# psweens/VAN-GAN

Measured on AMD Instinct MI355X. Metric: train Mvoxels/s (VanGan.train_step, 128^3 bf16), higher is better.
Workload: dtype bf16; 1 GPU; VanGan.train_step, 128x128x128 volumes, batch 1 per GPU (global 1), clDice on, disc noise+dropout on; parallelism=dp1

## Files before the change

### include/vangan_hip.h

```cpp
#ifndef VANGAN_HIP_H
#define VANGAN_HIP_H
#include <stdint.h>
#ifdef __cplusplus
extern "C" {
#endif

typedef void* vg_stream_t;

#define VG_OK 0
#define VG_EINVAL (-1)
#define VG_ELDS (-2)
#define VG_ELAUNCH (-3)

#define VG_ACT_NONE 0
#define VG_ACT_RELU 1
#define VG_ACT_LRELU 2

#define VG_PAD_ZERO 0
#define VG_PAD_REFLECT 1

#define VG_MAX_TAPS 64

#define VG_STRIPES 8

// ... 40 lines not shown
    int32_t Cout;
    const void* wpacked;
    int32_t CK;
    const float* bias;
    const void* res;
    const float* res_scale;
    const float* res_shift;
    int32_t tanh_out;
    void* out;
    int32_t out_f32;
    int32_t accumulate;
    float* out_sums;
    int32_t f32;
    int32_t nclass;
    int32_t cls_tap0[9];
    const void* cls_w[8];
    int32_t cls_ooff[8][3];
    int32_t cls_iters[8][3];
    int32_t wpack;
    int32_t wpack_wmin;
    const struct vg_actnorm_bwd_desc_s* bstat;
    void* scratch;
    int64_t scratch_bytes;
    int32_t wlayout;
    const vg_fin_desc* fin;
    int32_t res_c1;
    const void* wpacked_up;
} vg_conv_desc;
#define VG_SCRATCH_CTR_BYTES 16384

int vg_conv3d(const vg_conv_desc* d, vg_stream_t stream);

int vg_conv3d_lds_bytes(const vg_conv_desc* d);
int vg_conv3d_plan(const vg_conv_desc* d, int32_t* plan4);
int vg_conv3d_thin_np(const vg_conv_desc* d);
int vg_conv3d_variant(const vg_conv_desc* d, char* buf, int buflen);
int vg_set_tuning(const char* key, int value, int reset);

int vg_pack_up_weights(const float* w, int Cin, int Cout, int c_up, void* out, vg_stream_t stream);

int vg_pack_weights(const float* w, int T, int Cin, int Cout, const int32_t* tap_idx_dev, int ntaps,
                    int transpose, int CK, void* out, int out_f32, vg_stream_t stream);
typedef struct {
    const float* w; const int32_t* tap_idx; void* out;
    int32_t Cin, Cout, ntaps, transpose, CK, out_f32;
    int32_t blk0, nblk;
    int32_t bn;
    int32_t pad_;
} vg_pack_item;
int vg_pack_weights_multi(const vg_pack_item* items_dev, int n, int total_blocks, vg_stream_t stream);
int vg_conv3d_dma_bn(const vg_conv_desc* d);
int64_t vg_conv3d_scratch_bytes(const vg_conv_desc* d);
int vg_pack_weights_dma(const float* w, int T, int Cin, int Cout, const int32_t* tap_idx_dev, int ntaps, int transpose, int bn,
                        void* out, vg_stream_t stream);
int vg_packed_ktot(int ntaps, int C, int CK);
int vg_packed_rows(int N);

int vg_conv3d_wgrad(const vg_conv_desc* d, const void* dy, int dy_f32, const int32_t* tap_idx_host,
                    int T_total, float* dw, float* db, float* scratch, int64_t scratch_bytes, vg_stream_t stream);
int vg_conv3d_wgrad_variant(const vg_conv_desc* d, int dy_f32, const int32_t* tap_idx_host, int T_total,
                            int64_t scratch_bytes, char* buf, int buflen);

int vg_in_finalize(const float* sums0, int c0, float count0, const float* sums1, int c1, float count1,
                   const float* gamma, const float* beta, const float* mult, int N, float eps,
                   float* scale, float* shift, float* mean, float* rstd, vg_stream_t stream);

typedef struct vg_actnorm_bwd_desc_s {
    const void* g; int32_t g_padded;
    const void* x; int32_t x_f32;
    const void* x1; int32_t c_x0; int32_t x0_shift;
    int32_t N, D, H, W, C;
    const float* scale; const float* shift;
    const float* mult;
    int32_t act; int32_t norm;
    const float* gamma; const float* mean; const float* rstd;
    float* red;
    void* dx; int32_t dx_f32; int32_t accumulate;
    int32_t dx_cstride, dx_coff;
    int32_t f32;
    float* dgamma;
    float* dbeta;
    int32_t* ticket;
    int32_t alias_n0, alias_shift, pgrad_n, pad_;
} vg_actnorm_bwd_desc;
int vg_actnorm_bwd_stats(const vg_actnorm_bwd_desc* d, vg_stream_t stream);
int vg_actnorm_bwd_apply(const vg_actnorm_bwd_desc* d, vg_stream_t stream);
int vg_actnorm_bwd_apply2(const vg_actnorm_bwd_desc* d1, const vg_actnorm_bwd_desc* d2, vg_stream_t stream);
int vg_actnorm_bwd(const vg_actnorm_bwd_desc* d, vg_stream_t stream);
int vg_stem_short_fwd_workgroups(int N, int64_t S);
int vg_stem_short_fwd(const float* x, int N, int64_t S, int C, const float* w, const float* gamma, const float* beta, float eps, int round16,
                      float* scale, float* shift, double* part, int G, unsigned* ticket, vg_stream_t stream);
int vg_stem_short_bwd_workgroups(int N, int64_t S, int C);
int vg_stem_short_bwd(const void* g, int g_f32, const float* x, int N, int64_t S, int C, const float* w, const float* gamma, float eps,
                      int round16, float* dw, float* dgamma, float* dbeta, double* part, int G, unsigned* ticket, vg_stream_t stream);
int vg_in_param_grads(const float* red, int N, int C, float* dgamma, float* dbeta, vg_stream_t stream);

int vg_concat_bwd(const void* g, int N, int D, int H, int W, int Cu, int Cs, void* dlow, void* dskip,
                  int f32, int accumulate, vg_stream_t stream);

int vg_shortcut_dgrad_concat(const vg_conv_desc* d, void* dlow, void* dskip, int c_low, int accumulate, vg_stream_t stream);
int vg_shortcut_dgrad_concat_norm(const vg_conv_desc* d, const vg_actnorm_bwd_desc* b, void* dlow, void* dskip, int c_low,
                                  int accumulate, vg_stream_t stream);

int vg_affine_add(const void* a, const float* a_scale, const float* a_shift, int a_act, const void* b, const float* b_scale,
                  const float* b_shift, int N, int64_t S, int C, void* out, int f32, vg_stream_t stream);

int vg_bias_grad(const void* dy, int f32, int64_t rows, int C, float* db, vg_stream_t stream);

int vg_pack_cell_weights(const float* w, int C, void* out, vg_stream_t stream);
int vg_cells_fold(const void* cells, int N, int D, int H, int W, float* dx, vg_stream_t stream);

int vg_tanh_bwd(const float* dy, const float* y, float* dpre, int64_t n, vg_stream_t stream);

int vg_minmax(const float* x, int B, int64_t S, float* mm4, vg_stream_t stream);
int vg_minmax_apply(const float* x, const float* mm4, int B, int64_t S, float* y, vg_stream_t stream);
int vg_minmax_bwd(const float* x, const float* y, const float* gy, const float* mm4, int B, int64_t S,
                  float* tmp2, float* dx, vg_stream_t stream);
int vg_bce(const float* t, const float* p, int64_t n, float* acc, float gscale, float* gp, int accumulate,
           vg_stream_t stream);
int vg_mse(const float* a, const float* b, int64_t n, float* acc, float gscale, float* gb, int accumulate,
           vg_stream_t stream);
int vg_mse_const(const void* x, int x_f32, float target, int64_t n, float* acc, float gscale, float* gx,
                 int accumulate, vg_stream_t stream);
int vg_lp_loss(const float* a, const float* b, int64_t n, int p, float* acc, float gscale, float* gb, int accumulate,
               vg_stream_t stream);
int vg_logit_loss(const void* x, int x_f32, float target, int kind, int64_t n, float* acc, float gscale, float* gx,
                  int accumulate, vg_stream_t stream);
int vg_ssim_fwd(const float* t, const float* p, int B, int D, int H, int W, float* acc, float* part,
                vg_stream_t stream);
int vg_ssim_bwd(const float* t, const float* p, const float* part, int B, int D, int H, int W, float gscale,
                float* gp, int accumulate, vg_stream_t stream);

int vg_soft_skel_fwd(const float* img, int B, int D, int H, int W, int iters, float* imgs, float* skels, void* aux,
                     vg_stream_t stream);
int vg_soft_skel_bwd(const float* imgs, const float* skels, const float* gskel, int B, int D, int H, int W,
                     int iters, float* work, float* gimg, const void* aux, vg_stream_t stream);
int vg_cldice_coef(const float* sums7, float w, float alpha, float* coef6, vg_stream_t stream);
int vg_cldice_grads(const float* t, const float* skel_t, const float* coef6, int64_t n, float* gskel_p, float* gp,
                    int accumulate, vg_stream_t stream);
int vg_dot_sums(const float* a, const float* b, int64_t n, float* sums3, vg_stream_t stream);
int vg_axpby(const float* a, float alpha, const float* b, float beta, int64_t n, float* y, int accumulate,
             vg_stream_t stream);

int vg_dense_head_fwd(const float* x, const float* mask, const float* w, const float* b, int N, int n, float* z, vg_stream_t stream);
int vg_dense_head_bwd(const float* x, const float* mask, const float* w, const float* gz, int N, int n, float* dx, float* dw, float* db,
                      vg_stream_t stream);
int vg_wasserstein_terms(const float* z, int B, float inv, float* acc2, float* gz_d, float* gz_g, vg_stream_t stream);

int vg_overlap_add(const float* win, int kx, int ky, int kz, int px, int py, int pz, int x0, int y0, int z0,
                   int X, int Y, int Z, float* pred, float* cnt, vg_stream_t stream);
int vg_divide_crop(const float* pred, const float* cnt, int X, int Y, int Z, int sx, int sy, int sz, int ox, int oy,
                   int oz, float* out, vg_stream_t stream);
int vg_window_gather(const float* vol, int X, int Y, int Z, const int* tab, int B, int kx, int ky, int kz, float* out,
                     vg_stream_t stream);
int vg_window_scatter(const float* win, const int* tab, int B, int kx, int ky, int kz, int px, int py, int pz, const float* wx,
                      const float* wy, const float* wz, int X, int Y, int Z, float* pred, float* cnt, vg_stream_t stream);

int vg_adam_clip(float* w, const float* g, float* m, float* v, const int64_t* seg_off_dev, int T,
                 int64_t total, float* norms, float lr_t, float beta1, float beta2, float eps,
                 float clipnorm, float grad_scale, vg_stream_t stream);

#define VG_SN_MAX_ITEMS 8
#define VG_SN_MAX_PROJ 4
#define VG_SN_MAX_COUT 512
#define VG_SN_SLAB 65536
#define VG_SN_STATE 8
// ... 106 lines not shown
```

### van_gan_amd/_lib.py

```python
from __future__ import annotations

import ctypes as C
import os

import torch

from . import build as _build

VG_MAX_TAPS = 64
SN_STATE, SN_STATE_CUM, SN_MAX_PROJ = 8, 4, 4
ACT_NONE, ACT_RELU, ACT_LRELU = 0, 1, 2
PAD_ZERO, PAD_REFLECT = 0, 1
SCRATCH_CTR_BYTES = 16384

c_void_p, c_int, c_float, c_i64, c_u64 = C.c_void_p, C.c_int32, C.c_float, C.c_int64, C.c_uint64


class ConvDesc(C.Structure):
    _fields_ = [
        ('src0', c_void_p), ('src1', c_void_p), ('c_src0', c_int), ('c_src1', c_int), ('src0_shift', c_int),
        ('src_f32', c_int), ('N', c_int), ('D', c_int), ('H', c_int), ('W', c_int),
        ('in_scale', c_void_p), ('in_shift', c_void_p), ('act', c_int), ('noise', c_void_p), ('noise_pad', c_int),
        ('istr', c_int), ('pad_mode', c_int), ('ntaps', c_int),
        ('tap_d', C.c_int8 * VG_MAX_TAPS), ('tap_h', C.c_int8 * VG_MAX_TAPS), ('tap_w', C.c_int8 * VG_MAX_TAPS),
        ('OD', c_int), ('OH', c_int), ('OW', c_int), ('ostr', c_int), ('ooff_d', c_int), ('ooff_h', c_int),
        ('ooff_w', c_int), ('BD', c_int), ('BH', c_int), ('BW', c_int), ('Cout', c_int),
        ('wpacked', c_void_p), ('CK', c_int), ('bias', c_void_p),
        ('res', c_void_p), ('res_scale', c_void_p), ('res_shift', c_void_p), ('tanh_out', c_int),
        ('out', c_void_p), ('out_f32', c_int), ('accumulate', c_int), ('out_sums', c_void_p), ('f32', c_int),
        ('nclass', c_int), ('cls_tap0', c_int * 9), ('cls_w', c_void_p * 8), ('cls_ooff', (c_int * 3) * 8),
        ('cls_iters', (c_int * 3) * 8), ('wpack', c_int), ('wpack_wmin', c_int), ('bstat', c_void_p),
        ('scratch', c_void_p), ('scratch_bytes', c_i64), ('wlayout', c_int), ('fin', c_void_p), ('res_c1', c_int), ('wpacked_up', c_void_p),
    ]


class FinJob(C.Structure):
    _fields_ = [('gamma', c_void_p), ('beta', c_void_p), ('mult', c_void_p), ('scale', c_void_p), ('shift', c_void_p),
                ('mean', c_void_p), ('rstd', c_void_p), ('c_off', c_int), ('c_tot', c_int)]


class FinDesc(C.Structure):
    _fields_ = [('ticket', c_void_p), ('count', c_float), ('eps', c_float), ('njobs', c_int), ('job', FinJob * 2)]


class PackItem(C.Structure):
    _fields_ = [('w', c_void_p), ('tap_idx', c_void_p), ('out', c_void_p), ('Cin', c_int), ('Cout', c_int), ('ntaps', c_int),
                ('transpose', c_int), ('CK', c_int), ('out_f32', c_int), ('blk0', c_int), ('nblk', c_int), ('bn', c_int), ('pad_', c_int)]


class SnItem(C.Structure):
    _fields_ = [('w', c_void_p), ('u', c_void_p), ('state', c_void_p), ('K', c_int), ('Cout', c_int), ('blk0', c_int), ('nblk', c_int)]


class ActNormBwdDesc(C.Structure):
    _fields_ = [
        ('g', c_void_p), ('g_padded', c_int), ('x', c_void_p), ('x_f32', c_int),
        ('x1', c_void_p), ('c_x0', c_int), ('x0_shift', c_int),
        ('N', c_int), ('D', c_int), ('H', c_int), ('W', c_int), ('C', c_int),
        ('scale', c_void_p), ('shift', c_void_p), ('mult', c_void_p), ('act', c_int), ('norm', c_int),
        ('gamma', c_void_p), ('mean', c_void_p), ('rstd', c_void_p), ('red', c_void_p),
        ('dx', c_void_p), ('dx_f32', c_int), ('accumulate', c_int), ('dx_cstride', c_int), ('dx_coff', c_int),
        ('f32', c_int), ('dgamma', c_void_p), ('dbeta', c_void_p), ('ticket', c_void_p),
        ('alias_n0', c_int), ('alias_shift', c_int), ('pgrad_n', c_int), ('pad_', c_int),
    ]


_SIGS = {
    'vg_version': ([], c_int),
    'vg_storage16': ([], c_int),
    'vg_abi_sizeof': ([c_int], c_int),
    'vg_set_stamp_buffer': ([c_void_p], c_int),
    'vg_conv3d': ([C.POINTER(ConvDesc), c_void_p], c_int),
    'vg_conv3d_lds_bytes': ([C.POINTER(ConvDesc)], c_int),
    'vg_conv3d_plan': ([C.POINTER(ConvDesc), C.POINTER(C.c_int32)], c_int),
    'vg_conv3d_variant': ([C.POINTER(ConvDesc), C.c_char_p, c_int], c_int),
    'vg_conv3d_thin_np': ([C.POINTER(ConvDesc)], c_int),
    'vg_set_tuning': ([C.c_char_p, c_int, c_int], c_int),
    'vg_conv3d_wgrad_variant': ([C.POINTER(ConvDesc), c_int, C.POINTER(c_int), c_int, c_i64, C.c_char_p, c_int], c_int),
    'vg_pack_weights': ([c_void_p, c_int, c_int, c_int, c_void_p, c_int, c_int, c_int, c_void_p, c_int, c_void_p], c_int),
    'vg_pack_weights_multi': ([c_void_p, c_int, c_int, c_void_p], c_int),
    'vg_crop_augment': ([c_void_p] + [c_int] * 13 + [c_void_p, c_void_p], c_int),
    'vg_crop_max': ([c_void_p] + [c_int] * 10 + [c_void_p, c_void_p], c_int),
    'vg_conv3d_dma_bn': ([C.POINTER(ConvDesc)], c_int),
    'vg_conv3d_scratch_bytes': ([C.POINTER(ConvDesc)], c_i64),
    'vg_pack_weights_dma': ([c_void_p, c_int, c_int, c_int, c_void_p, c_int, c_int, c_int, c_void_p, c_void_p], c_int),
    'vg_packed_ktot': ([c_int, c_int, c_int], c_int),
    'vg_packed_rows': ([c_int], c_int),
    'vg_conv3d_wgrad': ([C.POINTER(ConvDesc), c_void_p, c_int, C.POINTER(c_int), c_int, c_void_p, c_void_p, c_void_p, c_i64,
                         c_void_p], c_int),
    'vg_in_finalize': ([c_void_p, c_int, c_float, c_void_p, c_int, c_float, c_void_p, c_void_p, c_void_p, c_int,
                        c_float, c_void_p, c_void_p, c_void_p, c_void_p, c_void_p], c_int),
    'vg_actnorm_bwd_stats': ([C.POINTER(ActNormBwdDesc), c_void_p], c_int),
    'vg_actnorm_bwd_apply': ([C.POINTER(ActNormBwdDesc), c_void_p], c_int),
    'vg_actnorm_bwd_apply2': ([C.POINTER(ActNormBwdDesc), C.POINTER(ActNormBwdDesc), c_void_p], c_int),
    'vg_actnorm_bwd': ([C.POINTER(ActNormBwdDesc), c_void_p], c_int),
    'vg_stem_short_fwd_workgroups': ([c_int, c_i64], c_int),
    'vg_stem_short_fwd': ([c_void_p, c_int, c_i64, c_int, c_void_p, c_void_p, c_void_p, C.c_float, c_int, c_void_p, c_void_p, c_void_p, c_int, c_void_p,
                          c_void_p], c_int),
    'vg_stem_short_bwd_workgroups': ([c_int, c_i64, c_int], c_int),
    'vg_stem_short_bwd': ([c_void_p, c_int, c_void_p, c_int, c_i64, c_int, c_void_p, c_void_p, C.c_float, c_int, c_void_p, c_void_p, c_void_p,
                          c_void_p, c_int, c_void_p, c_void_p], c_int),
    'vg_in_param_grads': ([c_void_p, c_int, c_int, c_void_p, c_void_p, c_void_p], c_int),
    'vg_concat_bwd': ([c_void_p, c_int, c_int, c_int, c_int, c_int, c_int, c_void_p, c_void_p, c_int, c_int, c_void_p], c_int),
    'vg_shortcut_dgrad_concat': ([C.POINTER(ConvDesc), c_void_p, c_void_p, c_int, c_int, c_void_p], c_int),
    'vg_shortcut_dgrad_concat_norm': ([C.POINTER(ConvDesc), C.POINTER(ActNormBwdDesc), c_void_p, c_void_p, c_int, c_int, c_void_p], c_int),
    'vg_affine_add': ([c_void_p, c_void_p, c_void_p, c_int, c_void_p, c_void_p, c_void_p, c_int, c_i64, c_int, c_void_p, c_int, c_void_p], c_int),
    'vg_bias_grad': ([c_void_p, c_int, c_i64, c_int, c_void_p, c_void_p], c_int),
    'vg_pack_cell_weights': ([c_void_p, c_int, c_void_p, c_void_p], c_int),
    'vg_cells_fold': ([c_void_p, c_int, c_int, c_int, c_int, c_void_p, c_void_p], c_int),
    'vg_tanh_bwd': ([c_void_p, c_void_p, c_void_p, c_i64, c_void_p], c_int),
    'vg_minmax': ([c_void_p, c_int, c_i64, c_void_p, c_void_p], c_int),
    'vg_minmax_apply': ([c_void_p, c_void_p, c_int, c_i64, c_void_p, c_void_p], c_int),
    'vg_minmax_bwd': ([c_void_p, c_void_p, c_void_p, c_void_p, c_int, c_i64, c_void_p, c_void_p, c_void_p], c_int),
    'vg_bce': ([c_void_p, c_void_p, c_i64, c_void_p, c_float, c_void_p, c_int, c_void_p], c_int),
    'vg_mse': ([c_void_p, c_void_p, c_i64, c_void_p, c_float, c_void_p, c_int, c_void_p], c_int),
    'vg_mse_const': ([c_void_p, c_int, c_float, c_i64, c_void_p, c_float, c_void_p, c_int, c_void_p], c_int),
    'vg_lp_loss': ([c_void_p, c_void_p, c_i64, c_int, c_void_p, c_float, c_void_p, c_int, c_void_p], c_int),
    'vg_logit_loss': ([c_void_p, c_int, c_float, c_int, c_i64, c_void_p, c_float, c_void_p, c_int, c_void_p], c_int),
    'vg_ssim_fwd': ([c_void_p, c_void_p, c_int, c_int, c_int, c_int, c_void_p, c_void_p, c_void_p], c_int),
    'vg_ssim_bwd': ([c_void_p, c_void_p, c_void_p, c_int, c_int, c_int, c_int, c_float, c_void_p, c_int, c_void_p], c_int),
    'vg_soft_skel_fwd': ([c_void_p, c_int, c_int, c_int, c_int, c_int, c_void_p, c_void_p, c_void_p, c_void_p], c_int),
    'vg_soft_skel_bwd': ([c_void_p, c_void_p, c_void_p, c_int, c_int, c_int, c_int, c_int, c_void_p, c_void_p, c_void_p, c_void_p], c_int),
    'vg_cldice_coef': ([c_void_p, c_float, c_float, c_void_p, c_void_p], c_int),
    'vg_cldice_grads': ([c_void_p, c_void_p, c_void_p, c_i64, c_void_p, c_void_p, c_int, c_void_p], c_int),
    'vg_dense_head_fwd': ([c_void_p, c_void_p, c_void_p, c_void_p, c_int, c_int, c_void_p, c_void_p], c_int),
    'vg_dense_head_bwd': ([c_void_p, c_void_p, c_void_p, c_void_p, c_int, c_int, c_void_p, c_void_p, c_void_p, c_void_p], c_int),
    'vg_wasserstein_terms': ([c_void_p, c_int, c_float, c_void_p, c_void_p, c_void_p, c_void_p], c_int),
    'vg_dot_sums': ([c_void_p, c_void_p, c_i64, c_void_p, c_void_p], c_int),
    'vg_overlap_add': ([c_void_p] + [c_int] * 12 + [c_void_p, c_void_p, c_void_p], c_int),
    'vg_divide_crop': ([c_void_p, c_void_p] + [c_int] * 9 + [c_void_p, c_void_p], c_int),
    'vg_window_gather': ([c_void_p, c_int, c_int, c_int, c_void_p] + [c_int] * 4 + [c_void_p, c_void_p], c_int),
    'vg_window_scatter': ([c_void_p, c_void_p] + [c_int] * 7 + [c_void_p] * 3 + [c_int] * 3 + [c_void_p] * 3, c_int),
    'vg_slice_moments_scratch_bytes': ([c_i64, c_int], c_i64),
    'vg_slice_moments': ([c_void_p, c_int, c_i64, c_int, c_void_p, c_void_p, c_i64, c_void_p], c_int),
    'vg_zscore_slices': ([c_void_p, c_int, c_i64, c_int, c_void_p, c_void_p, c_void_p, c_void_p], c_int),
    'vg_order_stats_scratch_bytes': ([c_i64, c_int], c_i64),
    'vg_order_stats': ([c_void_p, c_i64, C.POINTER(c_i64), c_int, c_void_p, c_void_p, c_i64, c_void_p], c_int),
    'vg_clip_rescale': ([c_void_p, c_i64, c_void_p, C.c_double, C.c_double, c_int, c_void_p, c_void_p, c_void_p], c_int),
    'vg_resample_axis': ([c_void_p, c_i64, c_int, c_i64, c_int, c_void_p, c_void_p, c_void_p, c_void_p], c_int),
    'vg_value_mode_scratch_bytes': ([c_i64], c_i64),
    'vg_value_mode': ([c_void_p, c_i64, c_void_p, c_void_p, c_void_p, c_i64, c_void_p], c_int),
    'vg_label_finish': ([c_void_p, c_i64, c_void_p, c_void_p, c_void_p, c_void_p, c_void_p], c_int),
    'vg_median3': ([c_void_p] + [c_int] * 7 + [c_void_p, c_void_p, c_void_p], c_int),
    'vg_volume_moments_scratch_bytes': ([c_i64], c_i64),
    'vg_volume_moments': ([c_void_p, c_int, c_i64, c_void_p, c_void_p, c_i64, c_void_p], c_int),
    'vg_outlier_limits': ([c_void_p, c_int, c_i64, c_void_p, c_float, c_void_p, c_void_p, c_void_p], c_int),
# ... 81 lines not shown
```

### van_gan_amd/csrc/vg_common.h

```cpp
#pragma once
#include <hip/hip_runtime.h>
#include <stdint.h>
#include "../../include/vangan_hip.h"

typedef __attribute__((ext_vector_type(8))) short bf16x8;
typedef __attribute__((ext_vector_type(4))) short bf16x4;
typedef __attribute__((ext_vector_type(4))) float f32x4;
typedef unsigned short bf16_t;

#define VG_LDS_LIMIT 163840
#define VG_LRELU 0.2f

#ifdef VG_FP16
typedef __attribute__((ext_vector_type(8))) _Float16 vg_h8;
__device__ __forceinline__ float bf2f(bf16_t h) { return (float)__builtin_bit_cast(_Float16, h); }
__device__ __forceinline__ bf16_t f2bf(float f) { return __builtin_bit_cast(unsigned short, (_Float16)f); }
#define VG_MFMA16(a, b, c) __builtin_amdgcn_mfma_f32_16x16x32_f16(__builtin_bit_cast(vg_h8, a), __builtin_bit_cast(vg_h8, b), c, 0, 0, 0)
#define VG_MFMA32(a, b, c) __builtin_amdgcn_mfma_f32_32x32x16_f16(__builtin_bit_cast(vg_h8, a), __builtin_bit_cast(vg_h8, b), c, 0, 0, 0)
#define VG_STORAGE16 "fp16"
#else
__device__ __forceinline__ float bf2f(bf16_t h) { return __uint_as_float(((unsigned)h) << 16); }
__device__ __forceinline__ bf16_t f2bf(float f) {
    __bf16 b = (__bf16)f;
    return __builtin_bit_cast(unsigned short, b);
// ... 36 lines not shown

__device__ __forceinline__ float vg_act(float x, int act) {
    if (act == VG_ACT_RELU) return fmaxf(x, 0.f);
    if (act == VG_ACT_LRELU) return x > 0.f ? x : VG_LRELU * x;
    return x;
}
__device__ __forceinline__ float vg_act_grad(float pre, int act) {
    if (act == VG_ACT_RELU) return pre > 0.f ? 1.f : 0.f;
    if (act == VG_ACT_LRELU) return pre > 0.f ? 1.f : VG_LRELU;
    return 1.f;
}

__device__ __forceinline__ float wave_sum(float v) {
#pragma unroll
    for (int o = 32; o > 0; o >>= 1) v += __shfl_xor(v, o);
    return v;
}
__device__ __forceinline__ float wave_min(float v) {
#pragma unroll
    for (int o = 32; o > 0; o >>= 1) v = fminf(v, __shfl_xor(v, o));
    return v;
}
__device__ __forceinline__ float wave_max(float v) {
#pragma unroll
    for (int o = 32; o > 0; o >>= 1) v = fmaxf(v, __shfl_xor(v, o));
    return v;
}

struct VgFin { unsigned* ticket; float count, eps; int njobs; vg_fin_job job[2]; };
static inline VgFin vg_fin_of(const vg_conv_desc* d) {
    VgFin f; f.ticket = nullptr; f.count = 1.f; f.eps = 0.f; f.njobs = 0;
    if (d->fin && d->out_sums) { f.ticket = d->fin->ticket; f.count = d->fin->count; f.eps = d->fin->eps; f.njobs = d->fin->njobs;
                                 f.job[0] = d->fin->job[0]; f.job[1] = d->fin->job[d->fin->njobs > 1 ? 1 : 0]; }
    return f;
}
__device__ __forceinline__ void vg_fin_one(const VgFin& f, float s, float ss, int n, int c) {
    const float mean = s / f.count;
    float var = ss / f.count - mean * mean;
    var = var < 0.f ? 0.f : var;
    const float rstd = rsqrtf(var + f.eps);
    for (int j = 0; j < f.njobs; ++j) {
        const vg_fin_job& q = f.job[j];
        const int cc = q.c_off + c, i = n * q.c_tot + cc;
        float sc = (q.gamma ? q.gamma[cc] : 1.f) * rstd;
        float sh = (q.beta ? q.beta[cc] : 0.f) - mean * sc;
        if (q.mult) { const float m = q.mult[i]; sc *= m; sh *= m; }
        q.scale[i] = sc; q.shift[i] = sh;
        if (q.mean) q.mean[i] = mean;
        if (q.rstd) q.rstd[i] = rstd;
    }
}
__device__ __forceinline__ void vg_fin_tail(const VgFin& f, const float* sums, int N, int C, unsigned nblocks, int* flag) {
    asm volatile("s_waitcnt vmcnt(0)" ::: "memory");
    __syncthreads();
    if (threadIdx.x == 0)
        *flag = __hip_atomic_fetch_add(f.ticket, 1u, __ATOMIC_RELAXED, __HIP_MEMORY_SCOPE_AGENT) == nblocks - 1u ? 1 : 0;
    __syncthreads();
    if (!*flag) return;
    for (int i = threadIdx.x; i < N * C; i += blockDim.x) {
        const int n = i / C, c = i - n * C;
        float s = 0.f, ss = 0.f;
        for (int t = 0; t < VG_STRIPES; ++t) {
            const float* p = sums + (((size_t)t * N + n) * C + c) * 2;
            s += __hip_atomic_load(p, __ATOMIC_RELAXED, __HIP_MEMORY_SCOPE_AGENT);
            ss += __hip_atomic_load(p + 1, __ATOMIC_RELAXED, __HIP_MEMORY_SCOPE_AGENT);
        }
        vg_fin_one(f, s, ss, n, c);
    }
}
int vg_launch_fin(const vg_conv_desc* d, hipStream_t s);
extern thread_local bool vg_fin_done;

int vg_tune(const char* key, int dflt);
bool vg_dry(const char* fmt, ...) __attribute__((format(printf, 1, 2)));
void vg_dry_begin(char* buf, int n);
void vg_dry_end();

bool vg_dry_on();
static inline void vg_begin() { (void)hipGetLastError(); }
static inline int vg_check_launch() {
    hipError_t e = hipGetLastError();
    return e == hipSuccess ? VG_OK : VG_ELAUNCH;
}
int vg_pointwise_conv(const vg_conv_desc* d, hipStream_t s);
int vg_pointwise_wgrad(const vg_conv_desc* d, const void* dy, int dy_f32, int T_total, float* dw, float* db, float* scratch,
                       int64_t scratch_bytes, hipStream_t s);
int vg_wgrad_dma(const vg_conv_desc* d, const void* dy, int dy_f32, const int32_t* tap_idx_host, int T_total, float* dw, float* db,
                 float* scratch, int64_t scratch_bytes, hipStream_t s);
int vg_wgrad_pw_dma(const vg_conv_desc* d, const void* dy, int dy_f32, int T_total, float* dw, float* db, float* scratch,
                    int64_t scratch_bytes, hipStream_t s);
int vg_wgrad_thin(const vg_conv_desc* d, const void* dy, int dy_f32, const int32_t* tap_idx_host, int T_total, float* dw, float* db,
                  float* scratch, int64_t scratch_bytes, hipStream_t s);
int vg_conv_dma(const vg_conv_desc* d, hipStream_t s, bool* did_stats = nullptr);
void vg_launch_reduce_partials(const float* part, int nb, int n, float* dw, hipStream_t s);
static inline int ilog2_exact(int v) { int l = 0; while ((1 << l) < v) ++l; return l; }
static inline int pow2_ceil(int v) { int p = 1; while (p < v) p <<= 1; return p; }
static inline int64_t cdiv64(int64_t a, int64_t b) { return (a + b - 1) / b; }

template <typename T> struct Raw8;
template <> struct Raw8<bf16_t> { bf16x8 v; };
template <> struct Raw8<float> { f32x4 a, b; };
__device__ __forceinline__ void raw_load(Raw8<bf16_t>& r, const bf16_t* p) { r.v = *(const __attribute__((address_space(1))) bf16x8*)(uintptr_t)p; }
__device__ __forceinline__ void raw_load(Raw8<float>& r, const float* p) {
    const __attribute__((address_space(1))) f32x4* q = (const __attribute__((address_space(1))) f32x4*)(uintptr_t)p;
    r.a = q[0]; r.b = q[1];
}
__device__ __forceinline__ void raw_unpack(const Raw8<bf16_t>& r, float* o) {
#pragma unroll
    for (int j = 0; j < 8; ++j) o[j] = bf2f((bf16_t)r.v[j]);
}
__device__ __forceinline__ void raw_unpack(const Raw8<float>& r, float* o) {
    o[0] = r.a[0]; o[1] = r.a[1]; o[2] = r.a[2]; o[3] = r.a[3]; o[4] = r.b[0]; o[5] = r.b[1]; o[6] = r.b[2]; o[7] = r.b[3];
}


__device__ __forceinline__ void raw_pin(Raw8<bf16_t>& r) { asm volatile("" : "+v"(r.v)); }
__device__ __forceinline__ void raw_pin(Raw8<float>& r) { asm volatile("" : "+v"(r.a), "+v"(r.b)); }
__device__ __forceinline__ void raw_mask(Raw8<bf16_t>& r, bool keep) { if (!keep) r.v = (bf16x8){0, 0, 0, 0, 0, 0, 0, 0}; }
__device__ __forceinline__ void raw_mask(Raw8<float>& r, bool keep) { if (!keep) { r.a = (f32x4){0.f, 0.f, 0.f, 0.f}; r.b = r.a; } }

__device__ __forceinline__ float ld_global(const float* p) { return *(const __attribute__((address_space(1))) float*)(uintptr_t)p; }
__device__ __forceinline__ float ld_global(const bf16_t* p) { return bf2f(*(const __attribute__((address_space(1))) bf16_t*)(uintptr_t)p); }
```

### van_gan_amd/csrc/vg_conv.hip

```cpp
#include "vg_conv_common.h"
#include "vg_dma_common.h"

unsigned long long* g_vg_stamps = nullptr;
extern "C" int vg_set_stamp_buffer(void* p) { g_vg_stamps = (unsigned long long*)p; return VG_OK; }
#define VG_STAMP(slot) do { if (g.stamps && tid == 0 && it < 8) g.stamps[((size_t)(blockIdx.z * gridDim.y + blockIdx.y) * gridDim.x + blockIdx.x) * 64 + it * 8 + (slot)] = __builtin_readcyclecounter(); } while (0)

__device__ __attribute__((aligned(16))) unsigned int vg_zero16[4];
typedef __attribute__((address_space(3))) void lds_void_t;
typedef const __attribute__((address_space(1))) void glb_void_t;

__device__ __forceinline__ void dma_build_cq(const GatherIn& g, int* cq, int tid) {
    const int SU = g.DS >> 4;
    for (int q = tid; q < SU; q += 256) {
        const int hh = q / g.HWp, hw = q - hh * g.HWp;
        cq[q] = (hh < g.HH && hw < g.HW) ? (hh | (hw << 10)) : -1;
    }
}
__device__ __forceinline__ void dma_build_tcol(const GatherIn& g, const int* cq, int* tcol, int oh0, int ow0, int tid) {
    const int SU = g.DS >> 4;
    const int ph0 = oh0 * g.istr + g.tmin_h, pw0 = ow0 * g.istr + g.tmin_w;
    const int sh = g.shift0, Ws0 = g.W >> sh;
    for (int q = tid; q < SU; q += 256) {
        const int e = cq[q];
        int o0 = -1, o1 = -1;
// ... 804 lines not shown
    if (!attr_set) {
        (void)hipFuncSetAttribute((const void*)conv_kernel<T, BN, MSUB, NOISE, WL, DMA, MC, C1>, hipFuncAttributeMaxDynamicSharedMemorySize, VG_LDS_LIMIT);
        attr_set = true;
    }
    const int wg_env = vg_tune("CONV_WGS", 0);
    int per_cu = ((BN / 16) * MSUB >= VG_CONV_MW2) ? 2 : VG_CONV_WAVES;
    if (lds > 0 && VG_LDS_LIMIT / lds < per_cu) per_cu = VG_LDS_LIMIT / lds;
    if (per_cu < 1) per_cu = 1;
    const int wg_target = wg_env > 0 ? wg_env : 256 * per_cu;
    const int tiles = g.tiles_d * g.tiles_h * g.tiles_w;
    const int ny = (k.Cout + BN - 1) / BN;
    const int ncp = MC == 2 ? q.ncls : 1;
    int bx = wg_target / (ny * g.N * ncp); if (bx < 1) bx = 1; if (bx > tiles) bx = tiles;
    int ks = 1;
    const long cells = (long)tiles * ny * g.N;
    const long ks_part_bytes = k.scratch_bytes - VG_SCRATCH_CTR_BYTES;
    if (MC == 0 && !DMA && !WL && k.nchunks > 1 && g.ntaps < VG_MAX_TAPS && bx == tiles && cells <= vg_tune("CONV_KSPLIT_CELLS", 256) && cells <= VG_KS_CELLS) {
        const int cap = vg_tune("CONV_KSPLIT", 8);
        constexpr long SLOTB = 256L * (MSUB * (BN / 16)) * 16;
        for (int c = k.nchunks; c >= 2; --c)
            if (k.nchunks % c == 0 && c <= cap && cells * c <= 1024 && cells * c * SLOTB <= ks_part_bytes) { ks = c; break; }
    }
    if (vg_dry("conv<%s,%d,%d,n%d,wl%d,dma%d,mc%d,c1%d>|walk%d|ch%d|ks%d", sizeof(T) == 4 ? "f32" : "bf16", BN, MSUB, (int)NOISE, (int)WL, (int)DMA,
               MC, (int)C1, tiles > bx ? 1 : 0, k.nchunks > 1 ? 1 : 0, ks)) return VG_OK;
    ConvOut k2 = k;
    k2.ks = ks; k2.ks_part = nullptr; k2.ks_cnt = nullptr;
    if (ks > 1) { k2.ks_cnt = (unsigned*)k.scratch; k2.ks_part = (float*)(k.scratch + VG_SCRATCH_CTR_BYTES); }
    dim3 grid(bx * ncp * ks, ny, g.N);
    hipLaunchKernelGGL((conv_kernel<T, BN, MSUB, NOISE, WL, DMA, MC, C1>), grid, dim3(256), lds, s, g, k2, q);
    if (k2.fin.ticket && k2.sums) vg_fin_done = true;
    return vg_check_launch();
}
template <typename T, int BN, int MSUB, bool NOISE>
static int launch_conv2(const GatherIn& g, const ConvOut& k, const ConvCls& q, int lds, hipStream_t s) {
    if (g.Cin == 1) {
        if (q.ncls > 1) return VG_EINVAL;
        if constexpr (sizeof(T) == 2) { if (k.w_lds) return launch_conv3<T, BN, MSUB, NOISE, true, false, 0, true>(g, k, q, lds, s); }
        return launch_conv3<T, BN, MSUB, NOISE, false, false, 0, true>(g, k, q, lds, s);
    }
    if constexpr (!NOISE) {
        if (q.par) {
            if constexpr (sizeof(T) == 2) { if (k.w_lds) return launch_conv3<T, BN, MSUB, NOISE, true, false, 2>(g, k, q, lds, s); }
            return launch_conv3<T, BN, MSUB, NOISE, false, false, 2>(g, k, q, lds, s);
        }
    }
    if constexpr (sizeof(T) == 2 && !NOISE) {
        if (q.ncls > 1) return k.w_lds ? launch_conv3<T, BN, MSUB, NOISE, true, false, 1>(g, k, q, lds, s)
                                       : launch_conv3<T, BN, MSUB, NOISE, false, false, 1>(g, k, q, lds, s);
        if (k.w_lds && k.dma) return launch_conv3<T, BN, MSUB, NOISE, true, true, 0>(g, k, q, lds, s);
    }
    if (q.ncls > 1) return VG_EINVAL;
    if constexpr (sizeof(T) == 2) { if (k.w_lds) return launch_conv3<T, BN, MSUB, NOISE, true, false, 0>(g, k, q, lds, s); }
    return launch_conv3<T, BN, MSUB, NOISE, false, false, 0>(g, k, q, lds, s);
}
template <typename T, int BN, int MSUB>
static int launch_conv(const GatherIn& g, const ConvOut& k, const ConvCls& q, int lds, hipStream_t s) {
    return g.noise ? launch_conv2<T, BN, MSUB, true>(g, k, q, lds, s) : launch_conv2<T, BN, MSUB, false>(g, k, q, lds, s);
}
template <typename T>
static int dispatch_conv(const GatherIn& g, const ConvOut& k, const ConvCls& q, int BN, int MSUB, int lds, hipStream_t s) {
    if (BN == 16 && MSUB == 8) { if constexpr (sizeof(T) == 2) return launch_conv<T, 16, 8>(g, k, q, lds, s); else return VG_EINVAL; }
    if (BN == 16) return MSUB == 4 ? launch_conv<T, 16, 4>(g, k, q, lds, s) : (MSUB == 2 ? launch_conv<T, 16, 2>(g, k, q, lds, s) : launch_conv<T, 16, 1>(g, k, q, lds, s));
    if (BN == 32) return MSUB == 4 ? launch_conv<T, 32, 4>(g, k, q, lds, s) : (MSUB == 2 ? launch_conv<T, 32, 2>(g, k, q, lds, s) : launch_conv<T, 32, 1>(g, k, q, lds, s));
    return MSUB == 2 ? launch_conv<T, 64, 2>(g, k, q, lds, s) : launch_conv<T, 64, 1>(g, k, q, lds, s);
}

static inline bool thin2_shape(const vg_conv_desc* d, const ConvOut& k, const ConvCls& q) {
    return !d->f32 && d->CK == 16 && d->Cout >= 32 && (d->Cout % 32) == 0 && q.ncls == 1 && d->ntaps == 27;
}

extern "C" int vg_conv3d_thin_np(const vg_conv_desc* d0) {
    vg_begin();
    if (!d0) return 0;
    vg_conv_desc d = *d0; d.CK = 16;
    GatherIn g, g2; ConvOut k; ConvCls q; int BN, MSUB, lds;
    if (fill_conv(&d, g, k, q, BN, MSUB, lds) != VG_OK || !thin2_shape(&d, k, q)) return 0;
    if (fill_gather(&d, g2, 16, 512) != VG_OK || !vg_conv_thin_ok(&d, g2, k, q, 2)) return 0;
    return vg_conv_thin_lds_bytes(g2, 2) <= VG_LDS_LIMIT ? 2 : 0;
}

static int conv3d_impl(const vg_conv_desc* d, vg_stream_t stream, bool& did_stats) {
    if (d && d->wlayout) return vg_conv_dma(d, (hipStream_t)stream, &did_stats);
    if (d && d->out && d->wpacked && d->src0 && !d->res_c1) {
        const int prc = vg_pointwise_conv(d, (hipStream_t)stream);
        if (prc <= 0) return prc;
    }
    GatherIn g; ConvOut k; ConvCls q; int BN, MSUB, lds;
    int rc = fill_conv(d, g, k, q, BN, MSUB, lds);
    if (rc != VG_OK) return rc;
    hipStream_t s = (hipStream_t)stream;
    if (!d->res_c1 && thin2_shape(d, k, q)) {
        GatherIn g2;
        if (fill_gather(d, g2, 16, 512) == VG_OK && vg_conv_thin_ok(d, g2, k, q, 2)) {
            const int trc = vg_launch_conv_thin(g2, k, 2, s, d->bstat ? d->bstat->red : nullptr, did_stats);
            if (trc <= 0 && trc != VG_ELDS) return trc;
        }
    }
    { GatherIn g2; int bn2, ms2, lds2; if (plan_conv32(d, k, q, g2, bn2, ms2, lds2) == VG_OK) return launch_conv32(g2, k, q, bn2, ms2, lds2, s); }
    if (!d->f32 && MSUB == 8 && BN == 16 && vg_conv_thin_ok(d, g, k, q, 1)) {
        const int trc = vg_launch_conv_thin(g, k, 1, s, d->bstat ? d->bstat->red : nullptr, did_stats);
        if (trc <= 0 && trc != VG_ELDS) return trc;
    }
    return d->f32 ? dispatch_conv<float>(g, k, q, BN, MSUB, lds, s) : dispatch_conv<bf16_t>(g, k, q, BN, MSUB, lds, s);
}

thread_local bool vg_fin_done = false;
__global__ void fin_kernel(VgFin f, const float* sums, int N, int C) {
    const int i = blockIdx.x * blockDim.x + threadIdx.x;
    if (i >= N * C) return;
    const int n = i / C, c = i - n * C;
    float s = 0.f, ss = 0.f;
    for (int t = 0; t < VG_STRIPES; ++t) { const float* p = sums + (((size_t)t * N + n) * C + c) * 2; s += p[0]; ss += p[1]; }
    vg_fin_one(f, s, ss, n, c);
}
int vg_launch_fin(const vg_conv_desc* d, hipStream_t s) {
    const VgFin f = vg_fin_of(d);
    if (!f.njobs) return VG_OK;
    const int total = d->N * d->Cout;
    hipLaunchKernelGGL(fin_kernel, dim3((total + 255) / 256), dim3(256), 0, s, f, (const float*)d->out_sums, d->N, d->Cout);
    return vg_check_launch();
}
static int fin_check(const vg_conv_desc* d) {
    const vg_fin_desc* f = d->fin;
    if (!f) return VG_OK;
    if (!d->out_sums || !f->ticket || f->njobs < 1 || f->njobs > 2 || !(f->count > 0.f)) return VG_EINVAL;
    for (int j = 0; j < f->njobs; ++j) {
        const vg_fin_job& q = f->job[j];
        if (!q.scale || !q.shift || q.c_off < 0 || q.c_off + d->Cout > q.c_tot) return VG_EINVAL;
    }
    return VG_OK;
}

extern "C" int vg_conv3d(const vg_conv_desc* d, vg_stream_t stream) {
    vg_begin();
    if (!d) return VG_EINVAL;
    if (fin_check(d) != VG_OK) return VG_EINVAL;
    vg_fin_done = false;
    const vg_actnorm_bwd_desc* b = d->bstat;
    if (b) {
        const int pd = b->g_padded ? 2 : 0;
        if (b->g != d->out || !b->norm || !b->red || !b->x || !b->mean || !b->rstd || b->f32 || d->f32 || d->out_f32 || d->accumulate
            || b->N != d->N || b->C != d->Cout || b->D + pd != d->BD || b->H + pd != d->BH || b->W + pd != d->BW)
            return VG_EINVAL;
    }
    bool did_stats = false;
    int rc = conv3d_impl(d, stream, did_stats);
    if (rc == VG_OK && d->fin && !vg_fin_done && !vg_dry_on()) rc = vg_launch_fin(d, (hipStream_t)stream);
    if (rc != VG_OK || !b || vg_dry_on()) return rc;
    if (did_stats) return rc;
    return vg_actnorm_bwd_stats(b, stream);
}

__global__ void pack_weights_kernel(const float* __restrict__ w, int Cin, int Cout, const int* __restrict__ tap_idx,
                                    int ntaps, int transpose, int CK, int kc_pad, int Ktot, int rows_pad,
                                    void* __restrict__ out, int out_f32) {
    const size_t total = (size_t)rows_pad * Ktot;
    const int NR = transpose ? Cin : Cout;
    const int C = transpose ? Cout : Cin;
    for (size_t i = (size_t)blockIdx.x * blockDim.x + threadIdx.x; i < total; i += (size_t)gridDim.x * blockDim.x) {
        const int row = (int)(i / Ktot), k = (int)(i % Ktot);
        const int chunk = k / kc_pad, kl = k % kc_pad;
        const int tap = kl / CK, ch = chunk * CK + kl % CK;
        float v = 0.f;
        if (row < NR && tap < ntaps && ch < C) {
            const int ts = tap_idx[tap];
            v = transpose ? w[((size_t)ts * Cin + row) * Cout + ch] : w[((size_t)ts * Cin + ch) * Cout + row];
        }
// ... 144 lines not shown
```

### van_gan_amd/csrc/vg_elem.hip

```cpp
#include "vg_common.h"
#include <stdlib.h>

__global__ void in_finalize_kernel(const float* sums0, int c0, float cnt0, const float* sums1, int c1, float cnt1,
                                   const float* gamma, const float* beta, const float* mult, int N, float eps,
                                   float* scale, float* shift, float* mean_o, float* rstd_o) {
    const int C = c0 + c1;
    const int i = blockIdx.x * blockDim.x + threadIdx.x;
    if (i >= N * C) return;
    const int n = i / C, c = i % C;
    float s = 0.f, ss = 0.f, cnt;
    if (c < c0) {
        for (int t = 0; t < VG_STRIPES; ++t) { s += sums0[(((size_t)t * N + n) * c0 + c) * 2]; ss += sums0[(((size_t)t * N + n) * c0 + c) * 2 + 1]; }
        cnt = cnt0;
    } else {
        for (int t = 0; t < VG_STRIPES; ++t) { s += sums1[(((size_t)t * N + n) * c1 + (c - c0)) * 2]; ss += sums1[(((size_t)t * N + n) * c1 + (c - c0)) * 2 + 1]; }
        cnt = cnt1;
    }
    const float mean = s / cnt;
    float var = ss / cnt - mean * mean;
    var = var < 0.f ? 0.f : var;
    const float rstd = rsqrtf(var + eps);
    float sc = (gamma ? gamma[c] : 1.f) * rstd;
    float sh = (beta ? beta[c] : 0.f) - mean * sc;
    if (mult) { const float m = mult[i]; sc *= m; sh *= m; }
    scale[i] = sc; shift[i] = sh;
    if (mean_o) mean_o[i] = mean;
    if (rstd_o) rstd_o[i] = rstd;
}

extern "C" int vg_in_finalize(const float* sums0, int c0, float count0, const float* sums1, int c1, float count1,
                              const float* gamma, const float* beta, const float* mult, int N, float eps,
                              float* scale, float* shift, float* mean, float* rstd, vg_stream_t stream) {
    vg_begin();
    if (!sums0 || c0 < 1 || c1 < 0 || (c1 > 0 && !sums1) || !scale || !shift || N < 1) return VG_EINVAL;
    const int total = N * (c0 + c1);
    hipLaunchKernelGGL(in_finalize_kernel, dim3((total + 255) / 256), dim3(256), 0, (hipStream_t)stream, sums0, c0,
                       count0, sums1, c1, count1, gamma, beta, mult, N, eps, scale, shift, mean, rstd);
    return vg_check_launch();
}

struct ANB {
    const void* g; int g_padded;
    const void* x; int x_f32;
    const void* x1; int c_x0, x0_shift;
    int N, D, H, W, C;
    const float* scale; const float* shift; const float* mult;
    int act, norm;
    const float* gamma; const float* mean; const float* rstd;
    float* red;
    int* ticket; float* dgamma; float* dbeta;
    void* dx; int dx_f32, accumulate, dx_cstride, dx_coff;
    int gpc, vpb;
    int alias_n0, alias_sh, pgrad_n;
};
__device__ __forceinline__ int anb_nx(const ANB& p, int n) { return (p.alias_n0 > 0 && n >= p.alias_n0) ? n - p.alias_sh : n; }

template <int VEC> struct ChanK { float sc[VEC], sh[VEC], mu[VEC], rs[VEC], ml[VEC]; };
__device__ __forceinline__ void ldvec(const float* p, float* o, int n) {
    if (n == 8) {
        const __attribute__((address_space(1))) f32x4* q = (const __attribute__((address_space(1))) f32x4*)(uintptr_t)p;
        const f32x4 a = q[0], b = q[1];
        o[0] = a[0]; o[1] = a[1]; o[2] = a[2]; o[3] = a[3]; o[4] = b[0]; o[5] = b[1]; o[6] = b[2]; o[7] = b[3];
    } else o[0] = *p;
}
template <int VEC>
__device__ __forceinline__ void load_chank(const ANB& p, int n, int c, ChanK<VEC>& k) {
    const int nc = anb_nx(p, n) * p.C + c;
#pragma unroll
    for (int j = 0; j < VEC; ++j) { k.sc[j] = 1.f; k.sh[j] = 0.f; k.mu[j] = 0.f; k.rs[j] = 0.f; k.ml[j] = 1.f; }
    if (p.scale) { ldvec(p.scale + nc, k.sc, VEC); ldvec(p.shift + nc, k.sh, VEC); }
    if (p.norm) { ldvec(p.mean + nc, k.mu, VEC); ldvec(p.rstd + nc, k.rs, VEC); }
    if (p.mult) ldvec(p.mult + nc, k.ml, VEC);
}

template <typename T, int VEC> struct RawV;
template <typename T> struct RawV<T, 8> { Raw8<T> r; };
template <typename T> struct RawV<T, 1> { float r; };
template <typename T> __device__ __forceinline__ void rawv_load(RawV<T, 8>& o, const T* p) { raw_load(o.r, p); }
template <typename T> __device__ __forceinline__ void rawv_load(RawV<T, 1>& o, const T* p) { o.r = ld_global(p); }
template <typename T> __device__ __forceinline__ void rawv_unpack(const RawV<T, 8>& o, float* v) { raw_unpack(o.r, v); }
template <typename T> __device__ __forceinline__ void rawv_unpack(const RawV<T, 1>& o, float* v) { v[0] = o.r; }

template <typename T, int VEC, int UB, typename F>
__device__ __forceinline__ void anb_walk_from(const ANB& p, int n, int c, int v, const int stride, const ChanK<VEC>& ck, F&& consume) {
    const int S = p.D * p.H * p.W;
    if (v >= S) return;
    int w = v % p.W, t0 = v / p.W; int h = t0 % p.H, d = t0 / p.H;
    const int sw = stride % p.W, t1 = stride / p.W; const int sh_ = t1 % p.H, sd = t1 / p.H;
    const int PH = p.H + 2, PW = p.W + 2;
    const T* gp = (const T*)p.g + (p.g_padded ? (size_t)n * (p.D + 2) * PH * PW * p.C : (size_t)n * S * p.C) + c;
    const bool need_x = p.act != VG_ACT_NONE || p.norm;
    const bool cat0 = p.x1 && c < p.c_x0;
    const int xs = p.x1 ? p.x0_shift : 0;
    const int Hs = p.H >> xs, Ws = p.W >> xs;
    const int cx = p.x1 ? (cat0 ? p.c_x0 : p.C - p.c_x0) : p.C;
    const T* xp = nullptr;
    const int nx = anb_nx(p, n);
    if (VEC == 8) xp = p.x1 ? (cat0 ? (const T*)p.x + (size_t)nx * (p.D >> xs) * Hs * Ws * cx + c : (const T*)p.x1 + (size_t)nx * S * cx + (c - p.c_x0))
                            : (const T*)p.x + (size_t)nx * S * cx + c;
    const void* x1p = (const char*)p.x + (size_t)nx * S * (p.x_f32 ? 4 : 2);
    for (; v < S; v += UB * stride) {
        RawV<T, VEC> gr[UB], xr[UB];
        float x1v[UB];
        int vv[UB], dd[UB], hh[UB], ww[UB];
#pragma unroll
        for (int k = 0; k < UB; ++k) {
            const bool ok = v + k * stride < S;
            vv[k] = ok ? v + k * stride : -1;
            dd[k] = d; hh[k] = h; ww[k] = w;
            const int vc = ok ? v + k * stride : v;
            const int dc = ok ? d : dd[0], hc = ok ? h : hh[0], wc = ok ? w : ww[0];
            const size_t gi = p.g_padded ? ((size_t)((dc + 1) * PH + hc + 1) * PW + wc + 1) * p.C : (size_t)vc * p.C;
            rawv_load(gr[k], gp + gi);
            if (need_x) {
                if (VEC == 8) {
                    const size_t xi = cat0 ? ((size_t)((dc >> xs) * Hs + (hc >> xs)) * Ws + (wc >> xs)) * cx : (size_t)vc * cx;
                    rawv_load(xr[k], xp + xi);
                } else {
                    x1v[k] = p.x_f32 ? ld_global((const float*)x1p + vc) : ld_global((const bf16_t*)x1p + vc);
                }
            }
            w += sw; if (w >= p.W) { w -= p.W; ++h; }
            h += sh_; if (h >= p.H) { h -= p.H; ++d; }
            d += sd;
        }
#pragma unroll
        for (int k = 0; k < UB; ++k) {
            if (vv[k] < 0) continue;
            float g[VEC], x[VEC];
            rawv_unpack(gr[k], g);
            if (need_x) { if (VEC == 8) rawv_unpack(xr[k], x); else x[0] = x1v[k]; }
            if (p.g_padded) {
                const int dk = dd[k], hk = hh[k], wk = ww[k];
                const bool dhb = dk == 1 || dk == p.D - 2 || hk == 1 || hk == p.H - 2;
                const bool wb = wk == 1 || wk == p.W - 2;
                if (dhb) {
                    const int md = dk == 1 ? 0 : (dk == p.D - 2 ? p.D + 1 : -1);
                    const int mh = hk == 1 ? 0 : (hk == p.H - 2 ? p.H + 1 : -1);
                    const int mw = wk == 1 ? 0 : (wk == p.W - 2 ? p.W + 1 : -1);
                    const int md2 = (dk == 1 && dk == p.D - 2) ? p.D + 1 : -1;
                    const int mh2 = (hk == 1 && hk == p.H - 2) ? p.H + 1 : -1;
                    const int mw2 = (wk == 1 && wk == p.W - 2) ? p.W + 1 : -1;
#pragma unroll
                    for (int a = 0; a < 3; ++a)
#pragma unroll
                        for (int b = 0; b < 3; ++b)
#pragma unroll
                            for (int e = 0; e < 3; ++e) {
                                if ((a | b | e) == 0) continue;
                                const int qd = a == 0 ? dk + 1 : (a == 1 ? md : md2);
                                const int qh = b == 0 ? hk + 1 : (b == 1 ? mh : mh2);
                                const int qw = e == 0 ? wk + 1 : (e == 1 ? mw : mw2);
                                if ((qd | qh | qw) < 0) continue;
                                const size_t idx = ((size_t)(qd * PH + qh) * PW + qw) * p.C;
                                if (VEC == 8) {
                                    float r[8]; load8<T>(gp + idx, r);
#pragma unroll
                                    for (int j = 0; j < 8; ++j) g[j] += r[j];
                                } else g[0] += ld1<T>(gp + idx);
                            }
                } else if (wb) {
                    const size_t rowi = (size_t)((dk + 1) * PH + hk + 1) * PW;
                    float r[VEC];
                    if (wk == 1) {
                        if (VEC == 8) load8<T>(gp + rowi * p.C, r); else r[0] = ld1<T>(gp + rowi * p.C);
#pragma unroll
                        for (int j = 0; j < VEC; ++j) g[j] += r[j];
                    }
                    if (wk == p.W - 2) {
                        if (VEC == 8) load8<T>(gp + (rowi + p.W + 1) * p.C, r); else r[0] = ld1<T>(gp + (rowi + p.W + 1) * p.C);
#pragma unroll
                        for (int j = 0; j < VEC; ++j) g[j] += r[j];
                    }
                }
            }
            float dn[VEC], xh[VEC];
            const float slope = p.act == VG_ACT_RELU ? 0.f : (p.act == VG_ACT_LRELU ? VG_LRELU : 1.f);
#pragma unroll
            for (int j = 0; j < VEC; ++j) {
                float gv = g[j] * ck.ml[j];
                if (need_x) {
                    const float pre = x[j] * ck.sc[j] + ck.sh[j];
                    gv *= (pre > 0.f || p.act == VG_ACT_NONE) ? 1.f : slope;
                    xh[j] = (x[j] - ck.mu[j]) * ck.rs[j];
                } else xh[j] = 0.f;
                dn[j] = gv;
            }
            consume(vv[k], dn, xh);
        }
    }
}

template <typename T, int VEC, int UB, typename F>
__device__ __forceinline__ void anb_walk(const ANB& p, int n, int c, int vl, const ChanK<VEC>& ck, F&& consume) {
    anb_walk_from<T, VEC, UB>(p, n, c, (int)(blockIdx.x * p.vpb + vl), (int)(gridDim.x * p.vpb), ck, consume);
}

template <typename T, int VEC>
__global__ __launch_bounds__(256) void actnorm_stats_kernel(const ANB p) {
    __shared__ float part[16 * 256];
    __shared__ float red[512 * 2];
    const int n = blockIdx.y;
    const int tid = threadIdx.x;
    const int nthr = p.gpc * p.vpb;
    const int cg = tid % p.gpc, vl = tid / p.gpc;
    float s0[VEC], s1[VEC];
#pragma unroll
    for (int j = 0; j < VEC; ++j) { s0[j] = 0.f; s1[j] = 0.f; }
    if (tid < nthr) {
        ChanK<VEC> ck;
        load_chank<VEC>(p, n, cg * VEC, ck);
        anb_walk<T, VEC, 4>(p, n, cg * VEC, vl, ck, [&](int, const float* dn, const float* xh) {
#pragma unroll
            for (int j = 0; j < VEC; ++j) { s0[j] += dn[j]; s1[j] += dn[j] * xh[j]; }
        });
    }
#pragma unroll
    for (int j = 0; j < VEC; ++j) { part[(2 * j) * 256 + tid] = tid < nthr ? s0[j] : 0.f; part[(2 * j + 1) * 256 + tid] = tid < nthr ? s1[j] : 0.f; }
    __syncthreads();
    for (int o = tid; o < p.C * 2; o += 256) {
        const int ch = o >> 1, mom = o & 1;
        const int g8 = ch / VEC, j = ch - g8 * VEC;
        const float* src = part + (2 * j + mom) * 256 + g8;
        float a = 0.f;
        for (int t = 0; t < p.vpb; ++t) a += src[t * p.gpc];
        red[o] = a;
    }
    __syncthreads();
    const int stripe = blockIdx.x & (VG_STRIPES - 1);
    float* dst = p.red + ((size_t)stripe * p.N + n) * p.C * 2;
    for (int i = tid; i < p.C * 2; i += 256) atomicAdd(&dst[i], red[i]);
}

template <typename T, int VEC>
__device__ __forceinline__ void actnorm_apply_body(const ANB& p, const int bx, const int gx) {
    const int n = blockIdx.y;
    const int tid = threadIdx.x;
    const int nthr = p.gpc * p.vpb;
    if (tid >= nthr) return;
    const int cg = tid % p.gpc, vl = tid / p.gpc;
    const int S = p.D * p.H * p.W;
    const int c = cg * VEC;
    float k0[VEC], k1[VEC], k2[VEC];
#pragma unroll
    for (int j = 0; j < VEC; ++j) { k0[j] = 1.f; k1[j] = 0.f; k2[j] = 0.f; }
    if (p.norm) {
        const int nc = n * p.C + c;
        const size_t total = (size_t)p.N * p.C * 2;
        float gm[VEC], rs[VEC], r[2 * VEC];
        ldvec(p.gamma + c, gm, VEC); ldvec(p.rstd + anb_nx(p, n) * p.C + c, rs, VEC);
#pragma unroll
        for (int j = 0; j < 2 * VEC; ++j) r[j] = 0.f;
#pragma unroll
        for (int t = 0; t < VG_STRIPES; ++t) {
            float q[2 * VEC];
            ldvec(p.red + t * total + (size_t)nc * 2, q, VEC);
            if (VEC == 8) ldvec(p.red + t * total + (size_t)nc * 2 + 8, q + 8, VEC); else q[1] = p.red[t * total + (size_t)nc * 2 + 1];
#pragma unroll
            for (int j = 0; j < 2 * VEC; ++j) r[j] += q[j];
        }
        if (p.dgamma && bx == 0 && vl == 0 && (p.pgrad_n <= 0 || n < p.pgrad_n)) {
#pragma unroll
            for (int j = 0; j < VEC; ++j) { atomicAdd(&p.dbeta[c + j], r[2 * j]); atomicAdd(&p.dgamma[c + j], r[2 * j + 1]); }
        }
        const float cnt = (float)S;
#pragma unroll
        for (int j = 0; j < VEC; ++j) { const float gr = gm[j] * rs[j]; k0[j] = gr; k1[j] = gr * r[2 * j] / cnt; k2[j] = gr * r[2 * j + 1] / cnt; }
    }
    ChanK<VEC> ck;
    load_chank<VEC>(p, n, c, ck);
    anb_walk_from<T, VEC, 4>(p, n, c, bx * p.vpb + vl, gx * p.vpb, ck, [&](int v, const float* dn, const float* xh) {
        float o[VEC];
#pragma unroll
        for (int j = 0; j < VEC; ++j) o[j] = k0[j] * dn[j] - k1[j] - k2[j] * xh[j];
        const size_t oidx = ((size_t)n * S + v) * p.dx_cstride + p.dx_coff + c;
        if (p.dx_f32) {
            float* q = (float*)p.dx + oidx;
#pragma unroll
            for (int j = 0; j < VEC; ++j) q[j] = p.accumulate ? q[j] + o[j] : o[j];
        } else if (VEC == 8) {
            bf16_t* q = (bf16_t*)p.dx + oidx;
            if (p.accumulate) {
                float old[8]; load8<bf16_t>(q, old);
#pragma unroll
                for (int j = 0; j < 8; ++j) o[j] += old[j];
            }
            store8<bf16_t>(q, o);
        } else {
            bf16_t* q = (bf16_t*)p.dx + oidx;
            q[0] = f2bf(p.accumulate ? bf2f(q[0]) + o[0] : o[0]);
        }
    });
}
template <typename T, int VEC>
__global__ __launch_bounds__(256) void actnorm_apply_kernel(const ANB p) { actnorm_apply_body<T, VEC>(p, (int)blockIdx.x, (int)gridDim.x); }
template <typename T, int VEC>
__global__ __launch_bounds__(256) void actnorm_apply2_kernel(const ANB p1, const ANB p2, const int g1) {
    if ((int)blockIdx.x < g1) actnorm_apply_body<T, VEC>(p1, (int)blockIdx.x, g1);
    else actnorm_apply_body<T, VEC>(p2, (int)blockIdx.x - g1, (int)gridDim.x - g1);
}

static int fill_anb(const vg_actnorm_bwd_desc* d, ANB& p, bool apply) {
    if (!d || !d->g || d->N < 1 || d->C < 1) return VG_EINVAL;
    if (d->C != 1 && (d->C % 8)) return VG_EINVAL;
    if (d->x_f32 && d->C != 1 && !d->f32) return VG_EINVAL;
    if ((d->act != VG_ACT_NONE || d->norm) && !d->x) return VG_EINVAL;
    if (d->norm && (!d->mean || !d->rstd || !d->red)) return VG_EINVAL;
    if (apply && (!d->dx || (d->norm && !d->gamma))) return VG_EINVAL;
    if (d->g_padded && (d->D < 2 || d->H < 2 || d->W < 2)) return VG_EINVAL;
    if (d->x1 && (d->C == 1 || (d->c_x0 % 8) || d->c_x0 < 8 || d->c_x0 >= d->C)) return VG_EINVAL;
    p.g = d->g; p.g_padded = d->g_padded; p.x = d->x; p.x_f32 = (d->x_f32 || d->f32) ? 1 : 0;
    p.x1 = d->x1; p.c_x0 = d->c_x0; p.x0_shift = d->x1 ? (d->x0_shift ? 1 : 0) : 0;
    p.N = d->N; p.D = d->D; p.H = d->H; p.W = d->W; p.C = d->C;
    p.scale = d->scale; p.shift = d->shift; p.mult = d->mult; p.act = d->act; p.norm = d->norm;
    p.gamma = d->gamma; p.mean = d->mean; p.rstd = d->rstd; p.red = d->red;
    p.ticket = d->ticket; p.dgamma = (d->dgamma && d->dbeta) ? d->dgamma : nullptr; p.dbeta = d->dbeta;
    p.dx = d->dx; p.dx_f32 = (d->dx_f32 || d->f32) ? 1 : 0; p.accumulate = d->accumulate;
    p.dx_cstride = d->dx_cstride > 0 ? d->dx_cstride : d->C; p.dx_coff = d->dx_coff;
    p.alias_n0 = d->alias_n0; p.alias_sh = d->alias_shift; p.pgrad_n = d->pgrad_n;
    if (d->alias_n0 < 0 || (d->alias_n0 > 0 && (d->alias_shift < 1 || d->alias_shift > d->alias_n0 || d->alias_n0 >= d->N)) || d->pgrad_n < 0) return VG_EINVAL;
    p.gpc = d->C == 1 ? 1 : d->C / 8;
    if (p.gpc > 256 || d->C > 512) return VG_EINVAL;
    p.vpb = 256 / p.gpc;
    if (!p.dx_f32 && d->C != 1 && ((p.dx_cstride % 8) || (p.dx_coff % 8))) return VG_EINVAL;
    return VG_OK;
}
static dim3 anb_grid(const ANB& p, bool stats = false) {
    const int S = p.D * p.H * p.W;
    int bx = (S + p.vpb - 1) / p.vpb;
    const int cap_total = vg_tune("ANB_GRID_CAP", 767), cap_stats = vg_tune("ANB_STATS_CAP", 511);
    int cap = (stats ? cap_stats : cap_total) / (p.N > 0 ? p.N : 1);
    if (cap < 1) cap = 1;
    if (bx > cap) bx = cap;
    return dim3(bx, p.N);
}

extern "C" int vg_actnorm_bwd_stats(const vg_actnorm_bwd_desc* d, vg_stream_t stream) {
    vg_begin();
    ANB p; int rc = fill_anb(d, p, false);
    if (rc != VG_OK) return rc;
    if (!p.red) return VG_EINVAL;
    if (d->f32) {
        if (p.C == 1) hipLaunchKernelGGL((actnorm_stats_kernel<float, 1>), anb_grid(p, true), dim3(256), 0, (hipStream_t)stream, p);
        else hipLaunchKernelGGL((actnorm_stats_kernel<float, 8>), anb_grid(p, true), dim3(256), 0, (hipStream_t)stream, p);
    } else {
        if (p.C == 1) hipLaunchKernelGGL((actnorm_stats_kernel<bf16_t, 1>), anb_grid(p, true), dim3(256), 0, (hipStream_t)stream, p);
        else hipLaunchKernelGGL((actnorm_stats_kernel<bf16_t, 8>), anb_grid(p, true), dim3(256), 0, (hipStream_t)stream, p);
    }
    return vg_check_launch();
}
extern "C" int vg_actnorm_bwd_apply(const vg_actnorm_bwd_desc* d, vg_stream_t stream) {
    vg_begin();
    ANB p; int rc = fill_anb(d, p, true);
    if (rc != VG_OK) return rc;
    if (d->f32) {
        if (p.C == 1) hipLaunchKernelGGL((actnorm_apply_kernel<float, 1>), anb_grid(p), dim3(256), 0, (hipStream_t)stream, p);
        else hipLaunchKernelGGL((actnorm_apply_kernel<float, 8>), anb_grid(p), dim3(256), 0, (hipStream_t)stream, p);
    } else {
        if (p.C == 1) hipLaunchKernelGGL((actnorm_apply_kernel<bf16_t, 1>), anb_grid(p), dim3(256), 0, (hipStream_t)stream, p);
        else hipLaunchKernelGGL((actnorm_apply_kernel<bf16_t, 8>), anb_grid(p), dim3(256), 0, (hipStream_t)stream, p);
    }
    return vg_check_launch();
}

extern "C" int vg_actnorm_bwd_apply2(const vg_actnorm_bwd_desc* d1, const vg_actnorm_bwd_desc* d2, vg_stream_t stream) {
    vg_begin();
    ANB p1, p2;
    int rc = fill_anb(d1, p1, true); if (rc != VG_OK) return rc;
    rc = fill_anb(d2, p2, true); if (rc != VG_OK) return rc;
    if (!vg_tune("ANB_APPLY2", 1) || d1->N != d2->N || (d1->f32 != 0) != (d2->f32 != 0) || d1->C == 1 || d2->C == 1) {
        rc = vg_actnorm_bwd_apply(d1, stream);
        return rc != VG_OK ? rc : vg_actnorm_bwd_apply(d2, stream);
    }
    const dim3 g1 = anb_grid(p1), g2 = anb_grid(p2);
    const dim3 grid(g1.x + g2.x, g1.y);
    if (d1->f32) hipLaunchKernelGGL((actnorm_apply2_kernel<float, 8>), grid, dim3(256), 0, (hipStream_t)stream, p1, p2, (int)g1.x);
    else hipLaunchKernelGGL((actnorm_apply2_kernel<bf16_t, 8>), grid, dim3(256), 0, (hipStream_t)stream, p1, p2, (int)g1.x);
    return vg_check_launch();
}

extern "C" int vg_actnorm_bwd(const vg_actnorm_bwd_desc* d, vg_stream_t stream) {
    if (d && d->norm) { const int rc = vg_actnorm_bwd_stats(d, stream); if (rc != VG_OK) return rc; }
    return vg_actnorm_bwd_apply(d, stream);
}

__global__ void in_param_grads_kernel(const float* red, int N, int C, float* dgamma, float* dbeta) {
    const int c = blockIdx.x * blockDim.x + threadIdx.x;
    if (c >= C) return;
    float a = 0.f, b = 0.f;
    for (int n = 0; n < N * VG_STRIPES; ++n) { a += red[((size_t)n * C + c) * 2]; b += red[((size_t)n * C + c) * 2 + 1]; }
    dbeta[c] += a; dgamma[c] += b;
}
template <typename T>
__global__ __launch_bounds__(256) void stem_short_bwd_kernel(const T* g, const float* x, int N, int64_t S, int C, const float* w, const float* gamma,
                                                             float eps, int round16, float* dw, float* dgamma, float* dbeta, double* part,
                                                             unsigned* ticket) {
    __shared__ float sm[4][8][18];
    __shared__ double fin[256][4];
    __shared__ int last;
    const int gpc = C >> 3, vpb = 256 / gpc, tid = threadIdx.x, cg = tid % gpc, vl = tid / gpc, n = blockIdx.y, G = gridDim.x, NV = 2 * C + 2;
    float r0[8], t[8], sx = 0.f, sxx = 0.f;
#pragma unroll
    for (int j = 0; j < 8; ++j) { r0[j] = 0.f; t[j] = 0.f; }
    const T* gn = g + (size_t)n * S * C + cg * 8;
    const float* xn = x + (size_t)n * S;
    constexpr int UN = 8;
    const int64_t vstep = (int64_t)G * vpb;
    int64_t v = (int64_t)blockIdx.x * vpb + vl;
    for (; v + (UN - 1) * vstep < S; v += UN * vstep) {
        Raw8<T> raw[UN]; float xv[UN];
#pragma unroll
        for (int u = 0; u < UN; ++u) { raw_load(raw[u], gn + (v + u * vstep) * C); xv[u] = ld_global(xn + v + u * vstep); }
#pragma unroll
        for (int u = 0; u < UN; ++u) {
            float gv[8];
            raw_unpack(raw[u], gv);
#pragma unroll
            for (int j = 0; j < 8; ++j) { r0[j] += gv[j]; t[j] = fmaf(gv[j], xv[u], t[j]); }
            sx += xv[u]; sxx = fmaf(xv[u], xv[u], sxx);
        }
    }
    for (; v < S; v += vstep) {
        float gv[8];
        load8<T>(gn + v * C, gv);
        const float xv = xn[v];
#pragma unroll
        for (int j = 0; j < 8; ++j) { r0[j] += gv[j]; t[j] = fmaf(gv[j], xv, t[j]); }
        sx += xv; sxx = fmaf(xv, xv, sxx);
    }
    float d[18];
#pragma unroll
    for (int j = 0; j < 8; ++j) { d[j] = r0[j]; d[8 + j] = t[j]; }
    d[16] = sx; d[17] = sxx;
    for (int o = 32; o >= gpc; o >>= 1) {
#pragma unroll
        for (int k = 0; k < 18; ++k) d[k] += __shfl_xor(d[k], o);
    }
    const int lane = tid & 63, wv = tid >> 6;
    if (lane < gpc) {
#pragma unroll
        for (int k = 0; k < 18; ++k) sm[wv][lane][k] = d[k];
    }
    __syncthreads();
    if (tid < NV) {
        int cgi, k;
        if (tid < C) { cgi = tid >> 3; k = tid & 7; }
        else if (tid < 2 * C) { cgi = (tid - C) >> 3; k = 8 + ((tid - C) & 7); }
        else { cgi = 0; k = 16 + tid - 2 * C; }
        __hip_atomic_store(part + ((size_t)n * G + blockIdx.x) * NV + tid,
                           (((double)sm[0][cgi][k] + (double)sm[1][cgi][k]) + (double)sm[2][cgi][k]) + (double)sm[3][cgi][k], __ATOMIC_RELAXED,
                           __HIP_MEMORY_SCOPE_AGENT);
    }
    asm volatile("s_waitcnt vmcnt(0)" ::: "memory");
    __syncthreads();
    if (tid == 0) last = __hip_atomic_fetch_add(ticket, 1u, __ATOMIC_RELAXED, __HIP_MEMORY_SCOPE_AGENT) == (unsigned)(N * G - 1) ? 1 : 0;
    __syncthreads();
    if (!last) return;
    auto ald = [](const double* q) { return __hip_atomic_load(q, __ATOMIC_RELAXED, __HIP_MEMORY_SCOPE_AGENT); };
// ... 544 lines not shown
```

### van_gan_amd/csrc/vg_pointwise.hip

```cpp
#include "vg_common.h"
#include "vg_c1k3.h"
#include <stdlib.h>

namespace {

struct PW {
    const void* x; int x_f32;
    const float* scale; const float* shift; int act;
    const void* w; int kc_pad, CK;
    const float* bias;
    void* out; int out_f32, accumulate, tanh_out;
    float* sums;
    const void* dy; int dy_f32;
    float* dw; float* db;
    int N, C; int64_t S;
    VgFin fin;
};

__device__ __forceinline__ float pw_slope(int act) { return act == VG_ACT_RELU ? 0.f : (act == VG_ACT_LRELU ? VG_LRELU : 1.f); }
__device__ __forceinline__ float ld_single(const void* p, int f32, int64_t i) {
    return f32 ? ld_global((const float*)p + i) : ld_global((const bf16_t*)p + i);
}

template <typename T, int G>
__global__ __launch_bounds__(256) void pw_cto1_kernel(const PW p) {
    const int n = blockIdx.y;
    float wv[G * 8], sc[G * 8], sf[G * 8];
#pragma unroll
    for (int c = 0; c < G * 8; ++c) {
        wv[c] = ld1<T>((const T*)p.w + (c / p.CK) * p.kc_pad + (c % p.CK));
        sc[c] = p.scale ? p.scale[n * p.C + c] : 1.f;
        sf[c] = p.scale ? p.shift[n * p.C + c] : 0.f;
    }
    const float slope = pw_slope(p.act), b = p.bias ? p.bias[0] : 0.f;
    const T* xb = (const T*)p.x + (size_t)n * p.S * p.C;
    const int64_t stride = (int64_t)gridDim.x * 256;
    float s1 = 0.f, s2 = 0.f;
    for (int64_t v = (int64_t)blockIdx.x * 256 + threadIdx.x; v < p.S; v += 2 * stride) {
        Raw8<T> r[2][G];
#pragma unroll
        for (int k = 0; k < 2; ++k) {
            const int64_t vv = v + k * stride < p.S ? v + k * stride : v;
#pragma unroll
            for (int g = 0; g < G; ++g) raw_load(r[k][g], xb + vv * p.C + g * 8);
        }
#pragma unroll
        for (int k = 0; k < 2; ++k) {
            if (v + k * stride >= p.S) continue;
            float a = b;
#pragma unroll
            for (int g = 0; g < G; ++g) {
                float x[8]; raw_unpack(r[k][g], x);
#pragma unroll
                for (int j = 0; j < 8; ++j) {
                    float y = x[j] * sc[g * 8 + j] + sf[g * 8 + j];
                    y = fmaxf(y, y * slope);
                    a += rnd<T>(y) * wv[g * 8 + j];
                }
            }
            const size_t o = (size_t)n * p.S + v + k * stride;
            if (p.tanh_out && !p.accumulate) a = tanhf(a);
            if (p.out_f32) { float* q = (float*)p.out + o; a = p.accumulate ? *q + a : a; *q = a; }
            else { bf16_t* q = (bf16_t*)p.out + o; const bf16_t h = f2bf(p.accumulate ? bf2f(*q) + a : a); *q = h; a = bf2f(h); }
            s1 += a; s2 += a * a;
        }
    }
    if (p.sums) {
        __shared__ float red[8];
#pragma unroll
        for (int o = 32; o > 0; o >>= 1) { s1 += __shfl_xor(s1, o); s2 += __shfl_xor(s2, o); }
        if ((threadIdx.x & 63) == 0) { red[(threadIdx.x >> 6) * 2] = s1; red[(threadIdx.x >> 6) * 2 + 1] = s2; }
        __syncthreads();
        if (threadIdx.x < 2) {
            const int stripe = blockIdx.x & (VG_STRIPES - 1);
            atomicAdd(&p.sums[((size_t)stripe * gridDim.y + n) * 2 + threadIdx.x],
                      red[threadIdx.x] + red[2 + threadIdx.x] + red[4 + threadIdx.x] + red[6 + threadIdx.x]);
        }
    }
}

template <typename T>
__global__ __launch_bounds__(256) void pw_1toc_kernel(const PW p) {
    __shared__ float part[16 * 256];
    const int n = blockIdx.y, tid = threadIdx.x;
    const int gpc = p.C >> 3, vpb = 256 / gpc;
    const int cg = tid % gpc, vl = tid / gpc;
    const bool live = tid < gpc * vpb;
    float wv[8], bv[8], s1[8], s2[8];
#pragma unroll
    for (int j = 0; j < 8; ++j) {
        wv[j] = live ? ld1<T>((const T*)p.w + (size_t)(cg * 8 + j) * p.kc_pad) : 0.f;
        bv[j] = (live && p.bias) ? p.bias[cg * 8 + j] : 0.f;
        s1[j] = 0.f; s2[j] = 0.f;
    }
    const float sc = p.scale ? p.scale[n] : 1.f, sf = p.scale ? p.shift[n] : 0.f, slope = pw_slope(p.act);
    const int64_t xoff = (int64_t)n * p.S;
    T* ob = (T*)p.out + (size_t)n * p.S * p.C + cg * 8;
    const int64_t stride = (int64_t)gridDim.x * vpb;
    if (live)
    for (int64_t v = (int64_t)blockIdx.x * vpb + vl; v < p.S; v += 4 * stride) {
        float xs[4]; Raw8<T> old[4];
#pragma unroll
        for (int k = 0; k < 4; ++k) {
            const int64_t vv = v + k * stride < p.S ? v + k * stride : v;
            xs[k] = ld_single(p.x, p.x_f32, xoff + vv);
            if (p.accumulate) raw_load(old[k], ob + vv * p.C);
        }
#pragma unroll
        for (int k = 0; k < 4; ++k) {
            if (v + k * stride >= p.S) continue;
            float y = xs[k] * sc + sf;
            y = rnd<T>(fmaxf(y, y * slope));
            float o[8];
#pragma unroll
            for (int j = 0; j < 8; ++j) o[j] = y * wv[j] + bv[j];
            if (p.accumulate) {
                float q[8]; raw_unpack(old[k], q);
#pragma unroll
                for (int j = 0; j < 8; ++j) o[j] += q[j];
            }
            store8<T>(ob + (v + k * stride) * p.C, o);
#pragma unroll
            for (int j = 0; j < 8; ++j) { const float r = rnd<T>(o[j]); s1[j] += r; s2[j] += r * r; }
        }
    }
    if (!p.sums) return;
#pragma unroll
    for (int j = 0; j < 8; ++j) { part[(2 * j) * 256 + tid] = live ? s1[j] : 0.f; part[(2 * j + 1) * 256 + tid] = live ? s2[j] : 0.f; }
    __syncthreads();
    const int stripe = blockIdx.x & (VG_STRIPES - 1);
    float* dst = p.sums + ((size_t)stripe * gridDim.y + n) * p.C * 2;
    for (int o = tid; o < p.C * 2; o += 256) {
        const int ch = o >> 1, mom = o & 1, g8 = ch >> 3, j = ch & 7;
        const float* src = part + (2 * j + mom) * 256 + g8;
        float a = 0.f;
        for (int t = 0; t < vpb; ++t) a += src[t * gpc];
        atomicAdd(&dst[o], a);
    }
    if (p.fin.ticket) vg_fin_tail(p.fin, p.sums, gridDim.y, p.C, gridDim.x * gridDim.y, (int*)part);
}

template <typename T, int GI>
__global__ __launch_bounds__(256) void pw_ctoc_kernel(const PW p, int Cin, int Ktot) {
    const int n = blockIdx.y, tid = threadIdx.x;
    const int gpc = p.C >> 3, vpb = 256 / gpc;
    const int cg = tid % gpc, vl = tid / gpc;
    if (tid >= gpc * vpb) return;
    float wv[GI * 8][8], bv[8];
#pragma unroll
    for (int k = 0; k < GI * 8; ++k)
#pragma unroll
        for (int j = 0; j < 8; ++j)
            wv[k][j] = ld1<T>((const T*)p.w + (size_t)(cg * 8 + j) * Ktot + (k / p.CK) * p.kc_pad + (k % p.CK));
#pragma unroll
    for (int j = 0; j < 8; ++j) bv[j] = p.bias ? p.bias[cg * 8 + j] : 0.f;
    const T* xb = (const T*)p.x + (size_t)n * p.S * Cin;
    T* ob = (T*)p.out + (size_t)n * p.S * p.C + cg * 8;
    const int64_t stride = (int64_t)gridDim.x * vpb;
    for (int64_t v = (int64_t)blockIdx.x * vpb + vl; v < p.S; v += 2 * stride) {
        Raw8<T> xr[2][GI], old[2];
#pragma unroll
        for (int k = 0; k < 2; ++k) {
            const int64_t vv = v + k * stride < p.S ? v + k * stride : v;
#pragma unroll
            for (int g = 0; g < GI; ++g) raw_load(xr[k][g], xb + vv * Cin + g * 8);
            if (p.accumulate) raw_load(old[k], ob + vv * p.C);
        }
#pragma unroll
        for (int k = 0; k < 2; ++k) {
            if (v + k * stride >= p.S) continue;
            float o[8];
#pragma unroll
            for (int j = 0; j < 8; ++j) o[j] = bv[j];
#pragma unroll
            for (int g = 0; g < GI; ++g) {
                float x[8]; raw_unpack(xr[k][g], x);
#pragma unroll
                for (int e = 0; e < 8; ++e)
#pragma unroll
                    for (int j = 0; j < 8; ++j) o[j] += x[e] * wv[g * 8 + e][j];
            }
            if (p.accumulate) {
                float q[8]; raw_unpack(old[k], q);
#pragma unroll
                for (int j = 0; j < 8; ++j) o[j] += q[j];
            }
            store8<T>(ob + (v + k * stride) * p.C, o);
        }
    }
}

struct PWG {
    const bf16_t* x0; const bf16_t* x1; int c0, c1, Cin, sh;
    const bf16_t* w; int Ktot, CK, kc_pad;
    const float* bias; bf16_t* out; float* sums;
    int N, ID, IH, IW, OD, OH, OW, istr;
    int BD, BH, BW, ostr, od0, oh0, ow0;
    int Cout; int SO;
    unsigned long long* stamps;
    bf16_t* dlow; bf16_t* dskip; int sc0, sacc;
    const bf16_t* ng; const bf16_t* nx0; const bf16_t* nx1;
    const float* n_scale; const float* n_shift; const float* n_mean; const float* n_rstd; const float* n_gamma; const float* n_mult;
    VgFin fin;
    const float* n_red; float* n_dgamma; float* n_dbeta; int n_act;
};
}
extern unsigned long long* g_vg_stamps;
// ... 716 lines not shown
        if (!nb_->norm || !nb_->g_padded || nb_->f32 || nb_->x_f32 || !nb_->g || !nb_->x || !nb_->x1 || !nb_->x0_shift || nb_->c_x0 != c_low) return 1;
        if (nb_->C != d->Cout || nb_->N != d->N || nb_->D != d->D || nb_->H != d->H || nb_->W != d->W || !nb_->gamma || !nb_->mean || !nb_->rstd || !nb_->red) return 1;
        if (d->D < 4 || d->H < 4 || d->W < 4 || d->D > 1023 || d->H > 1023 || d->W > 1023) return 1;
    }
    if (c_low < 16 || (c_low % 16) || c_low >= d->Cout) return 1;
    if (d->istr != 1 || d->ostr != 1 || d->ooff_d || d->ooff_h || d->ooff_w || d->BD != d->OD || d->BH != d->OH || d->BW != d->OW
        || d->OD != d->D || d->OH != d->H || d->OW != d->W || ((d->D | d->H | d->W) & 1)) return 1;
    const int64_t SO = (int64_t)d->OD * d->OH * d->OW;
    if (SO < 8 || SO > (1 << 30)) return 1;
    const int KS = (Cin + 31) / 32, NB = d->Cout / 16;
    if (!((KS == 1 && (NB == 3 || NB == 6)) || (KS == 2 && NB == 6))) return 1;
    PWG p = {};
    p.x0 = (const bf16_t*)d->src0; p.x1 = p.x0; p.c0 = Cin; p.c1 = 1; p.Cin = Cin; p.sh = 0;
    p.w = (const bf16_t*)d->wpacked; p.CK = d->CK; p.kc_pad = ((d->CK + 31) / 32) * 32; p.Ktot = ((Cin + d->CK - 1) / d->CK) * p.kc_pad;
    p.bias = nullptr; p.out = (bf16_t*)d->out; p.sums = nullptr;
    p.N = d->N; p.ID = d->D; p.IH = d->H; p.IW = d->W; p.OD = d->OD; p.OH = d->OH; p.OW = d->OW; p.istr = 1;
    p.BD = d->BD; p.BH = d->BH; p.BW = d->BW; p.ostr = 1;
    p.Cout = d->Cout; p.SO = (int)SO; p.stamps = g_vg_stamps;
    p.dlow = (bf16_t*)dlow; p.dskip = (bf16_t*)dskip; p.sc0 = c_low; p.sacc = acc;
    if (nb_) {
        p.ng = (const bf16_t*)nb_->g; p.nx0 = (const bf16_t*)nb_->x; p.nx1 = (const bf16_t*)nb_->x1;
        p.n_scale = nb_->scale; p.n_shift = nb_->shift; p.n_mean = nb_->mean; p.n_rstd = nb_->rstd; p.n_gamma = nb_->gamma; p.n_mult = nb_->mult;
        p.n_red = nb_->red; p.n_dgamma = (nb_->dgamma && nb_->dbeta) ? nb_->dgamma : nullptr; p.n_dbeta = nb_->dbeta; p.n_act = nb_->act;
    }
    const int MS = (KS * NB <= 2) ? 4 : 2;
    const int64_t nwt = (SO + MS * 16 - 1) / (MS * 16);
    int64_t b = (nwt + 3) / 4;
    const int capt = vg_tune("PW_GEMM_CAP", 2047);
    const int64_t cap = (capt / d->N) > 0 ? (capt / d->N) : 1;
    if (b > cap) b = cap;
    if (vg_dry("pw_gemm_split<%d,%d,n%d>", KS, NB, nb_ ? 1 : 0)) return VG_OK;
    const bool ok = nb_ ? pwg_launch_split<2>(KS, NB, dim3((int)b, d->N), s, p) : pwg_launch_split<1>(KS, NB, dim3((int)b, d->N), s, p);
    return ok ? vg_check_launch() : 1;
}

int pw_wgrad_cc(const vg_conv_desc* d, const void* dy, int dy_f32, int T_total, float* dw, float* db, float* scratch,
                int64_t scratch_bytes, hipStream_t s) {
    if (!pw_enabled() || !vg_tune("PW_WGRAD_CC", 1)) return 1;
    if (T_total != 1 || d->ntaps != 1 || d->tap_d[0] || d->tap_h[0] || d->tap_w[0] || d->noise || d->wpack || d->nclass > 1) return 1;
    if (d->f32 || d->src_f32 || dy_f32 || d->in_scale || d->act != VG_ACT_NONE) return 1;
    const int Cin = d->c_src0 + d->c_src1;
    if (Cin < 8 || (Cin % 8) || (d->c_src1 && (d->c_src0 % 8)) || d->Cout < 16 || (d->Cout % 16)) return 1;
    if (d->c_src1 && !d->src1) return 1;
    if (d->src0_shift && ((d->D | d->H | d->W) & 1)) return 1;
    if (d->istr < 1 || (d->OD - 1) * d->istr >= d->D || (d->OH - 1) * d->istr >= d->H || (d->OW - 1) * d->istr >= d->W) return 1;
    const int64_t SO = (int64_t)d->OD * d->OH * d->OW;
    if (SO < 1 || SO > (1 << 30)) return 1;
    PWW p = {};
    p.gin = Cin / 8; p.roles = p.gin * (d->Cout / 16);
    if (p.roles > vg_tune("PW_WGRAD_ROLES", 16)) return 1;
    p.rp = pow2_ceil(p.roles); p.vpb = 256 / p.rp;
    p.x0 = (const bf16_t*)d->src0; p.x1 = (const bf16_t*)(d->c_src1 ? d->src1 : d->src0); p.c0 = d->c_src0; p.c1 = d->c_src1 ? d->c_src1 : 1;
    p.Cin = Cin; p.sh = d->src0_shift ? 1 : 0; p.dy = (const bf16_t*)dy; p.Cout = d->Cout;
    p.N = d->N; p.ID = d->D; p.IH = d->H; p.IW = d->W; p.OD = d->OD; p.OH = d->OH; p.OW = d->OW; p.istr = d->istr; p.SO = (int)SO;
    p.dw = dw; p.db = db; p.dw_elems = Cin * d->Cout;
    int64_t b = (SO + (int64_t)p.vpb * 8 - 1) / ((int64_t)p.vpb * 8);
    const int capt = vg_tune("PW_WGRAD_CAP", 511);
    const int64_t cap = (capt / d->N) > 0 ? (capt / d->N) : 1;
    if (b > cap) b = cap;
    if (b < 1) b = 1;
    const int nslab = (int)b * d->N;
    p.part = (nslab > 4 && scratch && (int64_t)nslab * p.dw_elems * 4 <= scratch_bytes) ? scratch : nullptr;
    if (vg_dry("pw_wgrad_cc<r%d>|part%d", p.roles, p.part ? 1 : 0)) return VG_OK;
    hipLaunchKernelGGL(pw_wgrad_cc_kernel, dim3((int)b, d->N), dim3(256), 0, s, p);
    if (p.part) vg_launch_reduce_partials(p.part, nslab, p.dw_elems, dw, s);
    return vg_check_launch();
}

}

extern "C" int vg_shortcut_dgrad_concat(const vg_conv_desc* d, void* dlow, void* dskip, int c_low, int accumulate, vg_stream_t stream) {
    vg_begin();
    if (!d || !d->src0 || !d->out || !d->wpacked || !dlow || !dskip) return VG_EINVAL;
    return pw_gemm_split(d, nullptr, dlow, dskip, c_low, accumulate, (hipStream_t)stream);
}
extern "C" int vg_shortcut_dgrad_concat_norm(const vg_conv_desc* d, const vg_actnorm_bwd_desc* b, void* dlow, void* dskip, int c_low,
                                             int accumulate, vg_stream_t stream) {
    vg_begin();
    if (!d || !b || !d->src0 || !d->wpacked || !dlow || !dskip) return VG_EINVAL;
    if (!vg_tune("PW_SPLIT_NORM", 1)) return 1;
    return pw_gemm_split(d, b, dlow, dskip, c_low, accumulate, (hipStream_t)stream);
}

int vg_pointwise_conv(const vg_conv_desc* d, hipStream_t s) {
    if (pw_enabled() && !d->res && !d->tanh_out && !d->accumulate && d->ostr == 1 && !d->ooff_d && !d->ooff_h && !d->ooff_w
        && d->BD == d->OD && d->BH == d->OH && d->BW == d->OW && !(d->out_f32 && !d->f32)) {
        { const int mrc = c1m_fwd(d, s); if (mrc <= 0) return mrc; }
        C1K3 c;
        if (c1k3_fill(d, c)) {
            c.w = d->wpacked; c.bias = d->bias; c.out = d->out; c.sums = d->out_sums;
            c.fin = vg_fin_of(d);
            const int qpb = 256 / (c.C >> 3);
            int64_t b = ((int64_t)c.D * c.H * c.W4 + qpb - 1) / qpb;
            const int64_t cap = (2047 / d->N) > 0 ? (2047 / d->N) : 1;
            if (b > cap) b = cap;
            const dim3 grid((int)b, d->N);
            if (vg_dry("c1k3_fwd<%s,%s>", d->f32 ? "f32" : "bf16", d->src_f32 ? "f32" : "bf16")) return VG_OK;
            if (d->f32) {
                if (d->src_f32) hipLaunchKernelGGL((c1k3_fwd_kernel<float, float>), grid, dim3(256), 0, s, c);
                else hipLaunchKernelGGL((c1k3_fwd_kernel<float, bf16_t>), grid, dim3(256), 0, s, c);
            } else {
                if (d->src_f32) hipLaunchKernelGGL((c1k3_fwd_kernel<bf16_t, float>), grid, dim3(256), 0, s, c);
                else hipLaunchKernelGGL((c1k3_fwd_kernel<bf16_t, bf16_t>), grid, dim3(256), 0, s, c);
            }
            if (c.sums && c.fin.ticket) vg_fin_done = true;
            return vg_check_launch();
        }
    }
    { const int grc = pw_gemm_conv(d, s); if (grc <= 0) return grc; }
    if (!pw_shape_ok(d) || d->res) return 1;
    if (d->ostr != 1 || d->ooff_d || d->ooff_h || d->ooff_w || d->BD != d->OD || d->BH != d->OH || d->BW != d->OW) return 1;
    if (d->tanh_out && d->accumulate) return 1;
    const int Cin = d->c_src0;
    PW p = {};
    p.x = d->src0; p.x_f32 = d->src_f32; p.scale = d->in_scale; p.shift = d->in_shift; p.act = d->act;
    p.w = d->wpacked; p.CK = d->CK; p.kc_pad = ((d->CK + 31) / 32) * 32;
    p.bias = d->bias; p.out = d->out; p.out_f32 = (d->out_f32 || d->f32) ? 1 : 0; p.accumulate = d->accumulate; p.tanh_out = d->tanh_out;
    p.sums = d->out_sums; p.N = d->N; p.S = (int64_t)d->D * d->H * d->W;
    if (d->Cout == 1 && Cin >= 8 && Cin <= 32 && (Cin % 8) == 0) {
        p.C = Cin;
        const dim3 grid(pw_blocks((p.S + 1) / 2, d->N), d->N);
        if (vg_dry("pw_cto1<%s,%d>", d->f32 ? "f32" : "bf16", Cin / 8 > 4 ? 4 : Cin / 8)) return VG_OK;
#define PW_CTO1(T)                                                                                                      \
        switch (Cin / 8) {                                                                                              \
            case 1: hipLaunchKernelGGL((pw_cto1_kernel<T, 1>), grid, dim3(256), 0, s, p); break;                        \
            case 2: hipLaunchKernelGGL((pw_cto1_kernel<T, 2>), grid, dim3(256), 0, s, p); break;                        \
            case 3: hipLaunchKernelGGL((pw_cto1_kernel<T, 3>), grid, dim3(256), 0, s, p); break;                        \
            default: hipLaunchKernelGGL((pw_cto1_kernel<T, 4>), grid, dim3(256), 0, s, p); break;                       \
        }
        if (d->f32) { PW_CTO1(float) } else { PW_CTO1(bf16_t) }
#undef PW_CTO1
        return vg_check_launch();
    }
    if (Cin == 1 && d->Cout >= 8 && d->Cout <= 256 && (d->Cout % 8) == 0 && !d->tanh_out && !(d->out_f32 && !d->f32)) {
        p.C = d->Cout;
        p.kc_pad = ((d->CK + 31) / 32) * 32;
        const int vpb = 256 / (p.C >> 3);
        const dim3 grid(pw_blocks((p.S + 3) / 4 * (256 / vpb), d->N), d->N);
        if (vg_dry("pw_1toc<%s>", d->f32 ? "f32" : "bf16")) return VG_OK;
        p.fin = vg_fin_of(d);
        if (d->f32) hipLaunchKernelGGL((pw_1toc_kernel<float>), grid, dim3(256), 0, s, p);
        else hipLaunchKernelGGL((pw_1toc_kernel<bf16_t>), grid, dim3(256), 0, s, p);
        if (p.sums && p.fin.ticket) vg_fin_done = true;
        return vg_check_launch();
    }
    if ((Cin == 8 || Cin == 16) && d->Cout >= 16 && d->Cout <= 128 && (d->Cout % 8) == 0 && !d->in_scale && d->act == VG_ACT_NONE
        && !d->tanh_out && !d->out_sums && !d->src_f32 && !(d->out_f32 && !d->f32)) {
        p.C = d->Cout;
        const int nchunks = (Cin + d->CK - 1) / d->CK;
        const int Ktot = nchunks * p.kc_pad;
        const int vpb = 256 / (p.C >> 3);
        const dim3 grid(pw_blocks((p.S + 1) / 2 * (256 / vpb), d->N), d->N);
        if (vg_dry("pw_ctoc<%s,%d>", d->f32 ? "f32" : "bf16", Cin / 8)) return VG_OK;
        if (d->f32) {
            if (Cin == 8) hipLaunchKernelGGL((pw_ctoc_kernel<float, 1>), grid, dim3(256), 0, s, p, Cin, Ktot);
            else hipLaunchKernelGGL((pw_ctoc_kernel<float, 2>), grid, dim3(256), 0, s, p, Cin, Ktot);
        } else {
            if (Cin == 8) hipLaunchKernelGGL((pw_ctoc_kernel<bf16_t, 1>), grid, dim3(256), 0, s, p, Cin, Ktot);
            else hipLaunchKernelGGL((pw_ctoc_kernel<bf16_t, 2>), grid, dim3(256), 0, s, p, Cin, Ktot);
        }
        return vg_check_launch();
    }
    return 1;
}

int vg_pointwise_wgrad(const vg_conv_desc* d, const void* dy, int dy_f32, int T_total, float* dw, float* db, float* scratch,
                       int64_t scratch_bytes, hipStream_t s) {
    if (pw_enabled()) { const int mrc = c1m_wgrad(d, dy, dy_f32, T_total, dw, db, scratch, scratch_bytes, s); if (mrc <= 0) return mrc; }
    if (pw_enabled() && T_total == 9 && !(dy_f32 && !d->f32)) {
        C1K3 c;
        if (c1k3_fill(d, c)) {
            c.dy = dy; c.dw = dw; c.db = db;
            const int qpb = 256 / (3 * (c.C >> 3));
            int64_t b = ((int64_t)c.D * c.H * c.W4 + (int64_t)qpb * 8 - 1) / ((int64_t)qpb * 8);
            const int64_t cap = (767 / d->N) > 0 ? (767 / d->N) : 1;
            if (b > cap) b = cap;
            if (b < 1) b = 1;
            const dim3 grid((int)b, d->N);
            if (vg_dry("c1k3_wgrad<%s,%s>", d->f32 ? "f32" : "bf16", d->src_f32 ? "f32" : "bf16")) return VG_OK;
            if (d->f32) {
                if (d->src_f32) hipLaunchKernelGGL((c1k3_wgrad_kernel<float, float>), grid, dim3(256), 0, s, c);
                else hipLaunchKernelGGL((c1k3_wgrad_kernel<float, bf16_t>), grid, dim3(256), 0, s, c);
            } else {
                if (d->src_f32) hipLaunchKernelGGL((c1k3_wgrad_kernel<bf16_t, float>), grid, dim3(256), 0, s, c);
                else hipLaunchKernelGGL((c1k3_wgrad_kernel<bf16_t, bf16_t>), grid, dim3(256), 0, s, c);
            }
            return vg_check_launch();
        }
    }
    { const int wrc = pw_wgrad_cc(d, dy, dy_f32, T_total, dw, db, scratch, scratch_bytes, s); if (wrc <= 0) return wrc; }
    if (!pw_shape_ok(d) || T_total != 1) return 1;
    const int Cin = d->c_src0;
    PW p = {};
    p.x = d->src0; p.x_f32 = d->src_f32; p.scale = d->in_scale; p.shift = d->in_shift; p.act = d->act;
    p.dy = dy; p.dy_f32 = dy_f32; p.dw = dw; p.db = db; p.N = d->N; p.S = (int64_t)d->D * d->H * d->W;
    const bool c_to_1 = d->Cout == 1 && Cin >= 8 && Cin <= 256 && (Cin % 8) == 0;
    const bool one_to_c = Cin == 1 && d->Cout >= 8 && d->Cout <= 256 && (d->Cout % 8) == 0 && !(dy_f32 && !d->f32);
    if (!c_to_1 && !one_to_c) return 1;
    p.C = c_to_1 ? Cin : d->Cout;
    const int vpb = 256 / (p.C >> 3);
    int64_t b = (p.S + (int64_t)vpb * 16 - 1) / ((int64_t)vpb * 16);
    const int64_t cap = (511 / d->N) > 0 ? (511 / d->N) : 1;
    if (b > cap) b = cap;
    if (b < 1) b = 1;
    const dim3 grid((int)b, d->N);
    if (vg_dry("pw_wgrad<%s,%s>", d->f32 ? "f32" : "bf16", c_to_1 ? "cto1" : "1toc")) return VG_OK;
    if (c_to_1) {
        if (d->f32) hipLaunchKernelGGL((pw_wgrad_kernel<float, true>), grid, dim3(256), 0, s, p);
        else hipLaunchKernelGGL((pw_wgrad_kernel<bf16_t, true>), grid, dim3(256), 0, s, p);
    } else {
        if (d->f32) hipLaunchKernelGGL((pw_wgrad_kernel<float, false>), grid, dim3(256), 0, s, p);
        else hipLaunchKernelGGL((pw_wgrad_kernel<bf16_t, false>), grid, dim3(256), 0, s, p);
    }
    return vg_check_launch();
}
```

### van_gan_amd/nets.py

```python
from __future__ import annotations

import math
import os
from typing import Dict, List, Optional, Tuple

import torch

from . import ops
from .ops import ACT_LRELU, ACT_NONE, ACT_RELU, Arena, ConvLayer, Src

GEN_F = [16, 32, 64, 128, 256]
_STEM_AUX = os.environ.get('VG_STEM_AUX', '1') != '0'
_STEM_FUSED = os.environ.get('VG_STEM_FUSED', '1') != '0'


def gen_param_specs(attention_gate: bool = False) -> List[Tuple[str, Tuple[int, ...], str]]:
    f = GEN_F
    s: List[Tuple[str, Tuple[int, ...], str]] = []

    def conv(name, k, ci, co, init):
        s.append((name + '.w', (k, k, k, ci, co), init)); s.append((name + '.b', (co,), 'zeros'))

    def inorm(name, c):
        s.append((name + '.gamma', (c,), 'ones')); s.append((name + '.beta', (c,), 'zeros'))
# ... 353 lines not shown
            jobs['enc%d' % e] = [Nn['enc%d.cb1' % (e + 1)].job(pre['enc%d' % (e + 1)])] + dec_job(e, f[e + 1])
        jobs['enc4'] = [Nn['bridge.cb1'].job(pre['bridge.cb1'])]
        jobs['bridge.cb1'] = [Nn['bridge.cb2'].job(pre['bridge.cb2'])]
        jobs['bridge.cb2'] = dec_job(3)
        for d in (3, 2, 1):
            jobs['dec%d' % d] = dec_job(d - 1)
        jobs['dec0'] = None
        sx = Src(x, (N,) + lv[0], 1, f32=True)
        c1 = Act(ar, N, lv[0], f[0], dtype=self.dtype)
        L['stem.conv1'].forward(sx, c1.data, sums=c1.sums, fin=ops.fin_desc(ar, c1.count, [Nn['stem.cb'].job(pre['stem.cb'])]))
        fused = _STEM_FUSED and _STEM_AUX
        if fused:
            sc = None
            ns = dict(scale=ar.alloc((N, f[0]), torch.float32), shift=ar.alloc((N, f[0]), torch.float32), mean=None, rstd=None, mult=None)
            ops.stem_short_fwd(ar, x, N, f[0], L['stem.short'].w, Nn['stem.short'].gamma, Nn['stem.short'].beta, ns['scale'], ns['shift'],
                               round16=self.dtype != torch.float32)
        else:
            sc = Act(ar, N, lv[0], f[0], dtype=self.dtype)
            L['stem.short'].forward(sx, sc.data, sums=sc.sums, fin=ops.fin_desc(ar, sc.count, [Nn['stem.short'].job(pre['stem.short'])]))
            ns = pre['stem.short']
        n1 = pre['stem.cb']
        s1 = Src(c1.data, (N,) + lv[0], f[0], scale=n1['scale'], shift=n1['shift'], act=ACT_RELU)
        h = Act(ar, N, lv[0], f[0], dtype=self.dtype)
        L['stem.cb'].forward(s1, h.data, sums=h.sums, res=x if fused else sc.data, res_scale=ns['scale'], res_shift=ns['shift'],
                             fin=ops.fin_desc(ar, h.count, jobs['stem']), res_c1=fused)
        ctx['stem'] = dict(sx=sx, c1=c1, sc=sc, ns=ns, n1=n1, s1=s1, out=h)
        skips = [h]
        for e in range(1, 5):
            raw = Src(h.data, (N,) + lv[e - 1], f[e - 1])
            b = 'enc%d' % e
            h = self._block_fwd(ar, b, N, raw, pre[b], lv[e], f[e], ctx, save, out_jobs=jobs[b])
            if save:
                ctx['enc%d' % e]['inp'] = (skips[-1],)
            skips.append(h)
        nb1 = pre['bridge.cb1']
        sb1 = Src(h.data, (N,) + lv[4], f[4], scale=nb1['scale'], shift=nb1['shift'], act=ACT_RELU)
        b1 = Act(ar, N, lv[4], f[4], dtype=self.dtype)
        L['bridge.cb1'].forward(sb1, b1.data, sums=b1.sums, fin=ops.fin_desc(ar, b1.count, jobs['bridge.cb1']))
        nb2 = pre['bridge.cb2']
        sb2 = Src(b1.data, (N,) + lv[4], f[4], scale=nb2['scale'], shift=nb2['shift'], act=ACT_RELU)
        b2 = Act(ar, N, lv[4], f[4], dtype=self.dtype)
        L['bridge.cb2'].forward(sb2, b2.data, sums=b2.sums, fin=ops.fin_desc(ar, b2.count, jobs['bridge.cb2']) if jobs['bridge.cb2'] else None)
        ctx['bridge'] = dict(inp=h, nb1=nb1, sb1=sb1, b1=b1, nb2=nb2, sb2=sb2, b2=b2)
        h = b2
        for d in (3, 2, 1, 0):
            skip = skips[d]
            raw = Src(h.data, (N,) + lv[d], h.C, skip.data, skip.C, shift0=1)
            low = h
            b = 'dec%d' % d
            if self.attention_gate:
                out_pre = mkg = None
                if not save:
                    out_pre = Act(ar, N, lv[d], f[d], dtype=self.dtype)
                    mkg = ar.mark()
                gs, gctx = self._gate_fwd(ar, d, N, low, skip)
                raw = Src(low.data, (N,) + lv[d], low.C, gs.data, gs.C, shift0=1)
                n1 = Nn[b + '.cb1'].finalize(ar, low, gs)
                h = self._block_fwd(ar, b, N, raw, n1, lv[d], f[d], ctx, save, out_jobs=jobs[b], out=out_pre)
                if save:
                    ctx[b]['inp'] = (low, gs)
                    ctx[b]['gate'] = gctx
                else:
                    ar.release(mkg)
                continue
            h = self._block_fwd(ar, b, N, raw, pre[b], lv[d], f[d], ctx, save, out_jobs=jobs[b])
            if save:
                ctx['dec%d' % d]['inp'] = (low, skip)
        so = Src(h.data, (N,) + lv[0], f[0])
        L['out'].forward(so, y, tanh=True)
        ctx['out'] = dict(so=so, inp=h)
        return ctx

    def _norm_desc(self, ar, g, g_padded, src: Src, st, norm: Norm, dx, act, dx_cstride=0, accumulate=True):
        N = src.N
        red = ops.alloc_red(ar, N, src.C)
        return ops.actnorm_desc(g, g_padded, src.x0, (N, src.D, src.H, src.W), src.C, dx, scale=st['scale'], shift=st['shift'],
                                act=act, norm=True, gamma=norm.gamma, mean=st['mean'], rstd=st['rstd'], red=red,
                                accumulate=accumulate, x1=src.x1, c_x0=src.c0 if src.x1 is not None else 0, x0_shift=src.shift0,
                                dx_cstride=dx_cstride, dgamma=norm.dgamma, dbeta=norm.dbeta)

    def _norm_bwd(self, ar, g, g_padded, src: Src, st, norm: Norm, dx, act, dx_cstride=0, accumulate=True):
        ops.actnorm_run(self._norm_desc(ar, g, g_padded, src, st, norm, dx, act, dx_cstride, accumulate))

    def _dgrad_norm_bwd(self, ar, lay, dy, N, dp, src: Src, st, norm: Norm, dx, act, accumulate):
        dsc = self._norm_desc(ar, dp, True, src, st, norm, dx, act, accumulate=accumulate)
        ops.actnorm_run(dsc, stats_done=lay.dgrad(dy, N, dp, accumulate=False, bstat=dsc))

    def _block_bwd(self, ar: Arena, name: str, c: dict, N: int, inline: bool = False):
        L, Nn = self.L, self.Nn
        out, r, sc = c['out'], c['r'], c['sc']
        d_out = out.grad
        cb1, cb2, short = L[name + '.cb1'], L[name + '.cb2'], L[name + '.short']
        mk = ar.mark()
        d_sc = ar.alloc(sc.data.shape, self.dtype)
        ssc = Src(sc.data, (N,) + sc.dims, sc.C)
        dsc1 = self._norm_desc(ar, d_out, False, ssc, c['ns'], Nn[name + '.short'], d_sc, ACT_NONE, accumulate=False)
        ops.actnorm_stats(dsc1)
        cb2.wgrad(c['s2'], d_out, inline)
        dp = ar.alloc((N,) + cb2.buf_dims + (r.C,), self.dtype)
        d_r = ar.alloc(r.data.shape, self.dtype)
        dsc2 = self._norm_desc(ar, dp, True, c['s2'], c['n2'], Nn[name + '.cb2'], d_r, ACT_RELU, accumulate=False)
        if not cb2.dgrad(d_out, N, dp, accumulate=False, bstat=dsc2):
            ops.actnorm_stats(dsc2)
        ops.actnorm_apply2(dsc1, dsc2)
        s1, raw = c['s1'], c['src_raw']
        cb1.wgrad(s1, d_r, inline)
        short.wgrad(raw, d_sc, inline)
        dp1 = ar.alloc((N,) + cb1.buf_dims + (s1.C,), self.dtype)
        inp = c['inp']
        if len(inp) == 1:
            gin = inp[0].alloc_grad(ar) if inp[0].grad is None else inp[0].grad
            assert inp[0].grad_init, 'encoder input gradient must have had its first (overwriting) writer: the decoder skip path'
            self._dgrad_norm_bwd(ar, cb1, d_r, N, dp1, s1, c['n1'], Nn[name + '.cb1'], gin, ACT_RELU, accumulate=True)
            short.dgrad(d_sc, N, gin, accumulate=True)
        else:
            low, skip = inp
            dsc = self._norm_desc(ar, dp1, True, s1, c['n1'], Nn[name + '.cb1'], None, ACT_RELU, accumulate=False)
            stats_done = cb1.dgrad(d_r, N, dp1, accumulate=False, bstat=dsc)
            if not stats_done:
                ops.actnorm_stats(dsc)
            a_low, a_skip = not low.first_write(), not skip.first_write()
            if not short.dgrad_concat_norm(d_sc, N, dsc, low.C, low.grad, skip.grad, acc_low=a_low, acc_skip=a_skip):
                dcat = ar.alloc((N,) + tuple(cb1.in_dims) + (s1.C,), self.dtype)
                ops.actnorm_set_dx(dsc, dcat)
                ops.actnorm_run(dsc, stats_done=True)
                short.dgrad_concat(d_sc, N, dcat, low.C, low.grad, skip.grad, acc_low=a_low, acc_skip=a_skip)
        ar.release(mk, defer=True)

    def grad_suffix_offset(self, first_param: str = 'enc4.cb1.in.gamma') -> int:
        return self.store.offsets[first_param][0]

    def backward(self, ar: Arena, ctx: dict, gy: torch.Tensor, inline_from: int = -1, on_suffix_done=None):
        N = ctx['N']
        L, Nn = self.L, self.Nn
        acts = [ctx['stem']['out']] + [ctx['enc%d' % e]['out'] for e in range(1, 5)] + \
               [ctx['bridge']['b2']] + [ctx['dec%d' % d]['out'] for d in (3, 2, 1, 0)]
        if self.attention_gate:
            acts += [ctx['dec%d' % d]['inp'][1] for d in (3, 2, 1, 0)]
        for a in acts:
            a.grad = None
            a.alloc_grad(ar)
        dpre = ar.alloc(gy.shape, torch.float32)
        if isinstance(ctx['y'], list):
            nb = N // len(ctx['y'])
            for i, yi in enumerate(ctx['y']):
                ops.tanh_bwd(gy[i * nb:(i + 1) * nb], yi, dpre[i * nb:(i + 1) * nb])
        else:
            ops.tanh_bwd(gy, ctx['y'], dpre)
        h = ctx['out']['inp']
        L['out'].wgrad(ctx['out']['so'], dpre)
        L['out'].dgrad(dpre, N, h.grad, accumulate=not h.first_write())
        for d in (0, 1, 2, 3):
            self._block_bwd(ar, 'dec%d' % d, ctx['dec%d' % d], N)
            if self.attention_gate:
                self._gate_bwd(ar, d, ctx['dec%d' % d], N)
        b = ctx['bridge']
        mk = ar.mark()
        cb2, cb1 = L['bridge.cb2'], L['bridge.cb1']
        cb2.wgrad(b['sb2'], b['b2'].grad)
        dp = ar.alloc((N,) + cb2.buf_dims + (b['b1'].C,), self.dtype)
        d_b1 = ar.alloc(b['b1'].data.shape, self.dtype)
        self._dgrad_norm_bwd(ar, cb2, b['b2'].grad, N, dp, b['sb2'], b['nb2'], Nn['bridge.cb2'], d_b1, ACT_RELU, accumulate=False)
        cb1.wgrad(b['sb1'], d_b1)
        dp = ar.alloc((N,) + cb1.buf_dims + (b['inp'].C,), self.dtype)
        self._dgrad_norm_bwd(ar, cb1, d_b1, N, dp, b['sb1'], b['nb1'], Nn['bridge.cb1'], b['inp'].grad, ACT_RELU, accumulate=not b['inp'].first_write())
        ar.release(mk, defer=True)
        for e in (4, 3, 2, 1):
            self._block_bwd(ar, 'enc%d' % e, ctx['enc%d' % e], N, inline=e <= inline_from)
            if e == 4 and on_suffix_done is not None:
                on_suffix_done()
        inl = inline_from >= 0
        s = ctx['stem']
        d_out = s['out'].grad
        stem_aux = _STEM_AUX or s['sc'] is None
        ssc = None if s['sc'] is None else Src(s['sc'].data, (N,) + s['sc'].dims, s['sc'].C)
        if stem_aux:
            nrm = Nn['stem.short']
            ops.stem_short_bwd(ar, d_out, s['sx'].x0, N, GEN_F[0], L['stem.short'].w, nrm.gamma, L['stem.short'].gw,
                               dgamma=nrm.dgamma, dbeta=nrm.dbeta, round16=self.dtype != torch.float32)
        else:
            d_sc = ar.alloc(s['sc'].data.shape, self.dtype)
            self._norm_bwd(ar, d_out, False, ssc, s['ns'], Nn['stem.short'], d_sc, ACT_NONE, accumulate=False)
        cb = L['stem.cb']
        cb.wgrad(s['s1'], d_out, inl)
        dp = ar.alloc((N,) + cb.buf_dims + (s['c1'].C,), self.dtype)
        d_c1 = ar.alloc(s['c1'].data.shape, self.dtype)
        self._dgrad_norm_bwd(ar, cb, d_out, N, dp, s['s1'], s['n1'], Nn['stem.cb'], d_c1, ACT_RELU, accumulate=False)
        L['stem.conv1'].wgrad(s['sx'], d_c1, inl)
        if not stem_aux:
            L['stem.short'].wgrad(s['sx'], d_sc, inl)


RESNET_F, RESNET_DOWN, RESNET_RES, RESNET_UP = 32, 3, 6, 3


def resnet_param_specs() -> List[Tuple[str, Tuple[int, ...], str]]:
    s: List[Tuple[str, Tuple[int, ...], str]] = []

    def inorm(name, c):
        s.append((name + '.gamma', (c,), 'he_vec')); s.append((name + '.beta', (c,), 'zeros'))

    f = RESNET_F
    s.append(('c7.w', (7, 7, 7, 1, f), 'he_normal')); inorm('c7.in', f)
    for i in range(RESNET_DOWN):
        s.append(('down%d.w' % i, (3, 3, 3, f, 2 * f), 'he_normal')); inorm('down%d.in' % i, 2 * f)
        f *= 2
    for j in range(RESNET_RES):
        for c in ('c1', 'c2'):
            s.append(('res%d.%s.w' % (j, c), (3, 3, 3, f, f), 'he_normal')); inorm('res%d.%s.in' % (j, c), f)
    for i in range(RESNET_UP):
        s.append(('up%d.w' % i, (4, 4, 4, f, f // 2), 'he_normal')); inorm('up%d.in' % i, f // 2)
        f //= 2
    s.append(('out.w', (7, 7, 7, f, 1), 'glorot_uniform')); s.append(('out.b', (1,), 'zeros'))
    return s


class ResNetGenerator:

    def __init__(self, store: ParamStore, dims: Tuple[int, int, int], dtype: torch.dtype = torch.bfloat16):
        if any(n % 16 or n < 32 for n in dims):
            raise ValueError('spatial dims must be multiples of 16 and >= 32')
        self.dtype, self.store, self.dims = dtype, store, tuple(dims)
        L, Nn = {}, {}
        f = RESNET_F
        d = tuple(dims)
        L['c7'] = ConvLayer(store, 'c7', 7, 1, f, 1, 'reflect', False, d, need_dgrad=False, dtype=dtype)
        Nn['c7'] = Norm(store, 'c7.in', f)
        d = L['c7'].out_dims
        for i in range(RESNET_DOWN):
            k = 'down%d' % i
            L[k] = ConvLayer(store, k, 3, f, 2 * f, 2, 'reflect', False, d, need_dgrad=True, dtype=dtype)
            Nn[k] = Norm(store, k + '.in', 2 * f)
            d, f = L[k].out_dims, 2 * f
        for j in range(RESNET_RES):
            for c in ('c1', 'c2'):
                k = 'res%d.%s' % (j, c)
                L[k] = ConvLayer(store, k, 3, f, f, 1, 'reflect', False, d, need_dgrad=True, dtype=dtype)
                Nn[k] = Norm(store, k + '.in', f)
        for i in range(RESNET_UP):
            k = 'up%d' % i
            d = tuple(2 * n for n in d)
            L[k] = ConvLayer(store, k, 4, f, f // 2, 1, 'same', False, d, need_dgrad=True, dtype=dtype)
            Nn[k] = Norm(store, k + '.in', f // 2)
            f //= 2
        assert d == tuple(dims), (d, dims)
        self.head = [ConvLayer(store, 'out', 7, f, 1, 1, 'same', a == 0, d, need_dgrad=True, dtype=dtype,
                               tap_subset=list(range(a * 49, (a + 1) * 49))) for a in range(7)]
        self.L, self.Nn = L, Nn

    def pack(self):
        if getattr(self, '_ptab', None) is None:
# ... 321 lines not shown
```

### van_gan_amd/ops.py

```python
from __future__ import annotations

import ctypes as C
import os
import math
from typing import List, Optional, Sequence, Tuple

import torch

from . import _lib
from ._lib import ACT_LRELU, ACT_NONE, ACT_RELU, PAD_REFLECT, PAD_ZERO, ActNormBwdDesc, ConvDesc, FinDesc, check, lib

IN_EPS = 1e-3
STRIPES = 8


def _p(t: Optional[torch.Tensor]) -> Optional[int]:
    return None if t is None else t.data_ptr()


def conv_variant(d) -> str:
    buf = C.create_string_buffer(512)
    _lib.lib.vg_conv3d_variant(C.byref(d), buf, 512)
    return buf.value.decode()

# ... 186 lines not shown
        check(lib.vg_memset_zero(_p(t), t.numel() * t.element_size(), stream()), 'vg_memset_zero')


def copy(dst: torch.Tensor, src: torch.Tensor):
    if REC is None or not (dst.is_contiguous() and src.is_contiguous() and dst.dtype == src.dtype and dst.numel() == src.numel()):
        assert REC is None, 'recorded copies must be contiguous and type-preserving'
        dst.copy_(src)
    else:
        check(lib.vg_copy_bytes(_p(dst), _p(src), dst.numel() * dst.element_size(), stream()), 'vg_copy_bytes')


class Fp16:

    def __enter__(self):
        global lib
        self._saved = lib
        lib = _lib.lib_fp16()
        return self

    def __exit__(self, *exc):
        global lib
        lib = self._saved
        return False


class KernelProfile:

    def __init__(self):
        self.rows = {}
        self.vrows = {}
        self.lrows = {}

    def begin(self):
        e = torch.cuda.Event(enable_timing=True)
        e.record()
        return e

    def end(self, kind: str, flops: float, e0, nbytes: float = 0.0, variant: Optional[str] = None, layer: Optional[str] = None):
        e1 = torch.cuda.Event(enable_timing=True)
        e1.record()
        r = self.rows.setdefault(kind, [0, 0.0, [], 0.0])
        r[0] += 1; r[1] += flops; r[2].append((e0, e1)); r[3] += nbytes
        if variant:
            tmpl = variant.split('|')[0].replace(',bs1>', ',bs>').replace(',bs2>', ',bs>').replace(',bs1,pl>', ',bs,pl>').replace(',bs2,pl>', ',bs,pl>')
            v = self.vrows.setdefault((kind, tmpl), [0, 0.0, [], 0.0])
            v[0] += 1; v[1] += flops; v[2].append((e0, e1)); v[3] += nbytes
            if layer:
                v = self.lrows.setdefault((kind, layer, tmpl), [0, 0.0, [], 0.0])
                v[0] += 1; v[1] += flops; v[2].append((e0, e1)); v[3] += nbytes

    def by_layer(self):
        torch.cuda.synchronize()
        rows = []
        for (kind, layer, var), (n, fl, evs, nb) in self.lrows.items():
            ms = sum(a.elapsed_time(b) for a, b in evs)
            rows.append(dict(kind=kind, layer=layer, kernel=var, launches=n, ms=ms, gflop=fl / 1e9,
                             tflops=fl / (ms * 1e-3) / 1e12 if ms > 0 else None, algorithmic_bytes=nb))
        return sorted(rows, key=lambda r: -r['ms'])

    def summary(self):
        torch.cuda.synchronize()
        out = {}
        for k, (n, fl, evs, nb) in self.rows.items():
            ms = sum(a.elapsed_time(b) for a, b in evs)
            out[k] = dict(launches=n, flops=fl, ms=ms, bytes=nb)
        return out

    def by_variant(self):
        torch.cuda.synchronize()
        rows = []
        for (kind, var), (n, fl, evs, nb) in self.vrows.items():
            ms = sum(a.elapsed_time(b) for a, b in evs)
            rows.append(dict(kind=kind, kernel=var, launches=n, ms=ms, gflop=fl / 1e9, tflops=fl / (ms * 1e-3) / 1e12 if ms > 0 else None,
                             algorithmic_bytes=nb))
        return sorted(rows, key=lambda r: -r['ms'])


PROF: Optional[KernelProfile] = None

FUSE_CONCAT_NORM = os.environ.get('VG_FUSE_CONCAT_NORM', '1') != '0'
FUSE_CONCAT = os.environ.get('VG_FUSE_CONCAT', '1') != '0'
BSTAT = os.environ.get('VG_BSTAT', '1') != '0'
BSTAT_DMA = os.environ.get('VG_BSTAT_DMA', '0') != '0'
SIDE: Optional[bool] = None
_SIDE_OF = {}


def side_enable(device, on: bool = True):
    global SIDE
    SIDE = True if on else None


def _side_key(cur: torch.cuda.Stream):
    return (cur.device.index, cur.cuda_stream)


def _side_of(cur: torch.cuda.Stream) -> torch.cuda.Stream:
    sd = _SIDE_OF.get(_side_key(cur))
    if sd is None:
        sd = _SIDE_OF[_side_key(cur)] = torch.cuda.Stream(device=cur.device)
    return sd


class fork_side:

    def __init__(self):
        self.on = SIDE is not None and PROF is None and DRY is None
        self.cur = self.sd = self.ctx = None

    def __enter__(self):
        if self.on:
            self.cur = current_stream_obj()
            self.sd = _side_of(self.cur)
            wait_stream(self.sd, self.cur)
            self.ctx = torch.cuda.stream(self.sd)
            self.ctx.__enter__()
        return self

    def __exit__(self, *exc):
        if self.on:
            self.ctx.__exit__(*exc)
        return False

    def join(self):
        if self.on:
            wait_stream(self.cur, self.sd)


def side_event():
    if SIDE is None:
        return None
    sd = _SIDE_OF.get(_side_key(current_stream_obj()))
    return None if sd is None else record_event(sd)


def side_join():
    if SIDE is not None:
        cur = current_stream_obj()
        sd = _SIDE_OF.get(_side_key(cur))
        if sd is not None:
            wait_stream(cur, sd)


CONV_SCRATCH = {}
CONV_SCRATCH_BYTES = _lib.SCRATCH_CTR_BYTES + (int(os.environ.get('VG_CONV_SCRATCH_MB', '160')) << 20)
_SCRATCH_RETIRED = []


def conv_scratch(d: ConvDesc, s_: int, device=None):
    need = CONV_SCRATCH_BYTES
    if d.wlayout:
        need = max(need, int(lib.vg_conv3d_scratch_bytes(C.byref(d))))
    if DRY is not None:
        d.scratch, d.scratch_bytes = 1 << 20, need
        return
    key = (_DEV if device is None else device, s_)
    sc = CONV_SCRATCH.get(key)
    if sc is None or sc.numel() < need:
        dev = torch.device('cuda', key[0]) if key[0] is not None else torch.device('cuda')
        if sc is not None:
            _SCRATCH_RETIRED.append(sc)
        sc = torch.empty(need, dtype=torch.uint8, device=dev)
        sc[:_lib.SCRATCH_CTR_BYTES].zero_()
        CONV_SCRATCH[key] = sc
    d.scratch, d.scratch_bytes = sc.data_ptr(), sc.numel()

# ... 426 lines not shown
                                  dict(c_off=q.c_off, c_tot=q.c_tot, gamma=bool(q.gamma), beta=bool(q.beta), mult=bool(q.mult))
                                  for q in fin.job[:fin.njobs])))
        e0 = PROF.begin() if PROF is not None else None
        check(lib.vg_conv3d(C.byref(d), s_), 'vg_conv3d ' + self.name)
        if e0 is not None:
            esz = 4 if self.f32 else 2
            PROF.end('conv_fwd', 2.0 * src.N * math.prod(self.out_dims) * self.cout * self.cin * self.k ** 3, e0,
                     src.N * esz * (math.prod(self.in_dims) * self.cin + math.prod(self.out_dims) * self.cout), conv_variant(d), self.name)

    def wgrad(self, src: Src, dy: torch.Tensor, inline: bool = False):
        if SIDE is not None and PROF is None and DRY is None and not inline:
            cur = current_stream_obj()
            sd = _side_of(cur)
            wait_stream(sd, cur)
            self._wgrad(src, dy, sd.cuda_stream)
        else:
            self._wgrad(src, dy)

    def _wgrad(self, src: Src, dy: torch.Tensor, on_stream: Optional[int] = None):
        d = self._fwd_desc(src)
        s_ = stream() if on_stream is None else on_stream
        if DRY is not None:
            DRY.tag = ('wgrad', self.name)
            DRY.recipe = dict(kind='wgrad', layer=self.ctor, src=src.recipe(), dy_f32=dy.dtype == torch.float32)
        e0 = PROF.begin() if PROF is not None else None
        key = (dy.device, s_)
        sc = WGRAD_SCRATCH.get(key)
        if sc is None:
            sc = WGRAD_SCRATCH[key] = torch.empty(WGRAD_SCRATCH_ELEMS, dtype=torch.float32, device=dy.device)
        widx = self.f_idx_host if self.w_idx_host is None else self.w_idx_host
        check(lib.vg_conv3d_wgrad(C.byref(d), _p(dy), int(dy.dtype == torch.float32), widx, self.f_T,
                                  _p(self.gw_w), _p(self.gb), _p(sc), sc.numel() * 4, s_), 'vg_conv3d_wgrad ' + self.name)
        if e0 is not None:
            esz = 4 if self.f32 else 2
            vb = C.create_string_buffer(512)
            _lib.lib.vg_conv3d_wgrad_variant(C.byref(d), int(dy.dtype == torch.float32), widx, self.f_T, sc.numel() * 4, vb, 512)
            PROF.end('conv_wgrad', 2.0 * src.N * math.prod(self.out_dims) * self.cout * self.cin * self.k ** 3, e0,
                     src.N * esz * (math.prod(self.in_dims) * self.cin + math.prod(self.out_dims) * self.cout), vb.value.decode(), self.name)

    def _fused_desc(self, dy, N, out, accumulate, probe=False, plan=True):
        d = ConvDesc()
        dummy = 1 << 20
        d.src0, d.src1 = (dummy if probe else _p(dy)), None
        d.c_src0, d.c_src1, d.src0_shift = self.cout, 0, 0
        d.src_f32 = 0 if probe else int(dy.dtype == torch.float32 and self.cout == 1)
        d.N = N
        d.D, d.H, d.W = self.out_dims
        d.act, d.istr, d.pad_mode = ACT_NONE, 1, PAD_ZERO
        taps = [t for c in self.d_classes for t in c['taps']]
        _set_taps(d, taps)
        d.OD, d.OH, d.OW = [max(c['iters'][a] for c in self.d_classes) for a in range(3)]
        d.ostr = self.stride
        d.ooff_d, d.ooff_h, d.ooff_w = self.d_classes[0]['off']
        d.BD, d.BH, d.BW = self.buf_dims
        d.Cout, d.CK = self.cin, self.d_classes[0]['ck']
        d.f32 = self.f32
        d.nclass = len(self.d_classes)
        t0 = 0
        for i, c in enumerate(self.d_classes):
            d.cls_tap0[i] = t0
            t0 += len(c['taps'])
            d.cls_w[i] = dummy if probe else c['wp'].data_ptr()
            for a in range(3):
                d.cls_ooff[i][a] = c['off'][a]
                d.cls_iters[i][a] = c['iters'][a]
        d.cls_tap0[len(self.d_classes)] = t0
        d.wpacked = d.cls_w[0]
        d.wlayout = getattr(self, 'd_bn', 0)
        if probe and not plan:
            return d
        if probe:
            d.out = dummy
            plan = (C.c_int32 * 4)()
            ok = lib.vg_conv3d_plan(C.byref(d), plan) == 0
            self._last_plan = tuple(plan)
            return d if ok else None
        d.out, d.out_f32, d.accumulate = _p(out), int(out.dtype == torch.float32), int(accumulate)
        return d

    def dgrad(self, dy: torch.Tensor, N: int, out: torch.Tensor, accumulate: bool, bstat=None, bias=None) -> bool:
        use_bs = bstat is not None and BSTAT and not accumulate and not self.f32 and out.dtype in (torch.bfloat16, torch.float16) and bstat.norm \
            and ((len(self.d_classes) == 1 and self.stride == 1 and self.k == 3 and self.pad == 'reflect'
                  and self.d_classes[0]['ck'] == 16 and self.cin % 16 == 0 and self.cout % 16 == 0 and not bstat.mult)
                 or (bool(self.d_bn) and BSTAT_DMA))
        if DRY is not None:
            DRY.tag = ('dgrad', self.name)
            DRY.recipe = dict(kind='dgrad', layer=self.ctor, N=N, accumulate=bool(accumulate), dy_f32=dy.dtype == torch.float32,
                              out_f32=out.dtype == torch.float32, bstat=None if not use_bs else dict(
                                  cat=bool(bstat.x1), c_x0=bstat.c_x0, act=bstat.act, pad=bool(bstat.g_padded), mult=bool(bstat.mult),
                                  alias_n0=bstat.alias_n0, alias_shift=bstat.alias_shift))
        if REC is not None and use_bs:
            REC.keep.append(bstat)
        if self.d_fused:
            t = getattr(self, '_dg_tmpl', None)
            if t is None:
                t = self._dg_tmpl = self._fused_desc(dy, N, out, accumulate)
            d = ConvDesc()
            C.memmove(C.byref(d), C.byref(t), C.sizeof(ConvDesc))
            d.src0, d.N = _p(dy), N
            d.src_f32 = int(dy.dtype == torch.float32 and self.cout == 1)
            d.out, d.out_f32, d.accumulate = _p(out), int(out.dtype == torch.float32), int(accumulate)
            d.bstat = C.addressof(bstat) if use_bs else None
            d.bias = _p(bias)
            s_ = stream()
            conv_scratch(d, s_, out.device.index)
            e0 = PROF.begin() if PROF is not None else None
            check(lib.vg_conv3d(C.byref(d), s_), 'vg_conv3d(dgrad, fused classes) ' + self.name)
            if e0 is not None:
                PROF.end('conv_dgrad', 2.0 * N * math.prod(self.out_dims) * self.cin * self.cout * self.k ** 3, e0,
                         N * 2 * (math.prod(self.out_dims) * self.cout + math.prod(self.buf_dims) * self.cin), conv_variant(d), self.name)
            return use_bs
        for c in self.d_classes:
            t = c.get('tmpl')
            if t is None:
                t = ConvDesc()
                t.src1 = None
                t.c_src0, t.c_src1, t.src0_shift = self.cout, 0, 0
                t.D, t.H, t.W = self.out_dims
                t.act, t.istr, t.pad_mode = ACT_NONE, 1, PAD_ZERO
                _set_taps(t, c['taps'])
                t.OD, t.OH, t.OW = c['iters']
                t.ostr = self.stride
                t.ooff_d, t.ooff_h, t.ooff_w = c['off']
                t.BD, t.BH, t.BW = self.buf_dims
                t.Cout, t.wpacked, t.CK = self.cin, _p(c['wp']), c['ck']
                t.f32 = self.f32
                c['tmpl'] = t
            d = ConvDesc()
            C.memmove(C.byref(d), C.byref(t), C.sizeof(ConvDesc))
            d.src0, d.N = _p(dy), N
            d.src_f32 = int(dy.dtype == torch.float32 and self.cout == 1)
            d.out, d.out_f32, d.accumulate = _p(out), int(out.dtype == torch.float32), int(accumulate)
            d.bstat = C.addressof(bstat) if use_bs else None
            d.bias = _p(bias)
            s_ = stream()
            conv_scratch(d, s_, out.device.index)
            e0 = PROF.begin() if PROF is not None else None
            check(lib.vg_conv3d(C.byref(d), s_), 'vg_conv3d(dgrad) ' + self.name)
            if e0 is not None:
                PROF.end('conv_dgrad', 2.0 * N * math.prod(self.out_dims) * self.cin * self.cout * len(c['taps']), e0,
                         N * (4 if self.f32 else 2) * (math.prod(self.out_dims) * self.cout * len(c['taps']) / self.k ** 3
                                                       + math.prod(c['iters']) * self.cin), conv_variant(d), self.name)
        return use_bs


    def _sc_desc(self, dy, N):
        c = self.d_classes[0]
        d = ConvDesc()
        d.src1 = None
        d.c_src0, d.c_src1, d.src0_shift = self.cout, 0, 0
        d.D, d.H, d.W = self.out_dims
        d.act, d.istr, d.pad_mode = ACT_NONE, 1, PAD_ZERO
        _set_taps(d, c['taps'])
        d.OD, d.OH, d.OW = c['iters']
        d.ostr = self.stride
        d.ooff_d, d.ooff_h, d.ooff_w = c['off']
        d.BD, d.BH, d.BW = self.buf_dims
        d.Cout, d.wpacked, d.CK = self.cin, _p(c['wp']), c['ck']
        d.f32 = self.f32
        d.src0, d.N = _p(dy), N
        return d

    def dgrad_input(self, ar: 'Arena', dy: torch.Tensor, N: int, dx: torch.Tensor):
        assert self.cin == 1 and self.pad == 'reflect'
        if self.cell is None or DRY is not None or dy.dtype not in (torch.bfloat16, torch.float16):
            dp = ar.alloc((N,) + tuple(self.buf_dims) + (1,), self.dtype)
            self.dgrad(dy, N, dp, accumulate=False)
# ... 155 lines not shown
    def run(self, n_proj: int = 1):
        check(lib.vg_spectral_norm(_p(self.table), self.n, self.total_blocks, n_proj, _p(self.scratch), self.scratch.numel() * 4, stream()),
              'vg_spectral_norm')


def in_finalize(sums0, c0, count0, gamma, beta, N, scale, shift, mean=None, rstd=None, sums1=None, c1=0, count1=1.0,
                mult=None):
    check(lib.vg_in_finalize(_p(sums0), c0, float(count0), _p(sums1), c1, float(count1), _p(gamma), _p(beta), _p(mult),
                             N, IN_EPS, _p(scale), _p(shift), _p(mean), _p(rstd), stream()), 'vg_in_finalize')


def fin_desc(ar: 'Arena', count: float, jobs) -> FinDesc:
    f = FinDesc()
    tk = ar.alloc((1,), torch.int32, zero=True)
    f.ticket, f.count, f.eps, f.njobs = _p(tk), float(count), IN_EPS, len(jobs)
    keep = [tk]
    for j, (gamma, beta, mult, st, c_off, c_tot) in enumerate(jobs):
        q = f.job[j]
        q.gamma, q.beta, q.mult = _p(gamma), _p(beta), _p(mult)
        q.scale, q.shift, q.mean, q.rstd = _p(st['scale']), _p(st['shift']), _p(st['mean']), _p(st['rstd'])
        q.c_off, q.c_tot = c_off, c_tot
        keep += [gamma, beta, mult, st]
    f._keep = keep
    return f


def alloc_red(ar: 'Arena', N: int, C_: int) -> torch.Tensor:
    return ar.alloc((STRIPES * N * C_ * 2 + 4,), torch.float32, zero=True)


def actnorm_desc(g, g_padded, x, dims, C_, dx, *, scale=None, shift=None, mult=None, act=ACT_NONE, norm=False,
                 gamma=None, mean=None, rstd=None, red=None, accumulate=False, x1=None, c_x0=0, x0_shift=0,
                 dx_cstride=0, dx_coff=0, dgamma=None, dbeta=None, alias_n0=0, alias_shift=0, pgrad_n=0) -> ActNormBwdDesc:
    d = ActNormBwdDesc()
    d.g, d.g_padded = _p(g), int(g_padded)
    d.x, d.x_f32 = _p(x), int(x is not None and x.dtype == torch.float32)
    d.x1, d.c_x0, d.x0_shift = _p(x1), c_x0, x0_shift
    d.N, d.D, d.H, d.W = dims
    d.C = C_
    d.scale, d.shift, d.mult, d.act, d.norm = _p(scale), _p(shift), _p(mult), act, int(norm)
    d.gamma, d.mean, d.rstd, d.red = _p(gamma), _p(mean), _p(rstd), _p(red)
    d.dx, d.dx_f32, d.accumulate = _p(dx), int(dx is not None and dx.dtype == torch.float32), int(accumulate)
    d.dx_cstride, d.dx_coff = dx_cstride, dx_coff
    d.f32 = int(g.dtype == torch.float32)
    d.dgamma, d.dbeta = _p(dgamma), _p(dbeta)
    d.alias_n0, d.alias_shift, d.pgrad_n = alias_n0, alias_shift, pgrad_n
    nred = STRIPES * dims[0] * C_ * 2
    d.ticket = (red.data_ptr() + 4 * nred) if (red is not None and red.dim() == 1 and red.numel() == nred + 4) else None
    d._keep = (g, x, dx, scale, shift, mult, gamma, mean, rstd, red, x1, dgamma, dbeta)
    return d


def actnorm_stats(d: ActNormBwdDesc):
    check(lib.vg_actnorm_bwd_stats(C.byref(d), stream()), 'vg_actnorm_bwd_stats')


def stem_short_fwd(ar: 'Arena', x, N, C_, w, gamma, beta, scale, shift, round16=True):
    S = x.numel() // N
    G = int(lib.vg_stem_short_fwd_workgroups(N, S))
    if G < 1:
        raise _lib.VgError('vg_stem_short_fwd: unsupported shape N=%d S=%d' % (N, S))
    part = ar.alloc((N, G, 2), torch.float64)
    ticket = ar.alloc((4,), torch.int32, zero=True)
    check(lib.vg_stem_short_fwd(_p(x), N, S, C_, _p(w), _p(gamma), _p(beta), IN_EPS, int(round16), _p(scale), _p(shift), _p(part), G, _p(ticket),
                                stream()), 'vg_stem_short_fwd')


def stem_short_bwd(ar: 'Arena', g, x, N, C_, w, gamma, dw, dgamma=None, dbeta=None, round16=True):
    S = g.numel() // (N * C_)
    G = int(lib.vg_stem_short_bwd_workgroups(N, S, C_))
    if G < 1:
        raise _lib.VgError('vg_stem_short_bwd: unsupported shape N=%d S=%d C=%d' % (N, S, C_))
    part = ar.alloc((N, G, 2 * C_ + 2), torch.float64)
    ticket = ar.alloc((4,), torch.int32, zero=True)
    check(lib.vg_stem_short_bwd(_p(g), int(g.dtype == torch.float32), _p(x), N, S, C_, _p(w), _p(gamma), IN_EPS, int(round16), _p(dw), _p(dgamma),
                                _p(dbeta), _p(part), G, _p(ticket), stream()), 'vg_stem_short_bwd')


def actnorm_set_dx(d: ActNormBwdDesc, dx: torch.Tensor):
    d.dx, d.dx_f32 = _p(dx), int(dx.dtype == torch.float32)
    d._keep = d._keep + (dx,)


def actnorm_run(d: ActNormBwdDesc, stats_done: bool = False):
    if stats_done:
        check(lib.vg_actnorm_bwd_apply(C.byref(d), stream()), 'vg_actnorm_bwd_apply')
    else:
        check(lib.vg_actnorm_bwd(C.byref(d), stream()), 'vg_actnorm_bwd')


def actnorm_apply2(d1: ActNormBwdDesc, d2: ActNormBwdDesc):
    check(lib.vg_actnorm_bwd_apply2(C.byref(d1), C.byref(d2), stream()), 'vg_actnorm_bwd_apply2')


def actnorm_bwd(g, g_padded, x, dims, C_, dx, **kw):
    actnorm_run(actnorm_desc(g, g_padded, x, dims, C_, dx, **kw))


def concat_bwd(g, dims, Cu, Cs, dlow, dskip, acc_low: bool = True, acc_skip: bool = True):
    N, D, H, W = dims
    check(lib.vg_concat_bwd(_p(g), N, D, H, W, Cu, Cs, _p(dlow), _p(dskip), int(g.dtype == torch.float32),
                            int(bool(acc_low)) | (int(bool(acc_skip)) << 1), stream()), 'vg_concat_bwd')


def affine_add(a, a_scale, a_shift, a_act, b, b_scale, b_shift, N, S, C_, out):
    check(lib.vg_affine_add(_p(a), _p(a_scale), _p(a_shift), a_act, _p(b), _p(b_scale), _p(b_shift), N, S, C_, _p(out),
                            int(out.dtype == torch.float32), stream()), 'vg_affine_add')


def attn_gate_fwd(skip, phi, w_theta, b_theta, w_psi, b_psi, dims, Cs, Ci, gated, h, sums):
    N, D, H, W = dims
    check(lib.vg_attn_gate_fwd(_p(skip), _p(phi), _p(w_theta), _p(b_theta), _p(w_psi), _p(b_psi), N, D, H, W, Cs, Ci,
                               int(skip.dtype == torch.float32), _p(gated), _p(h), _p(sums), stream()), 'vg_attn_gate_fwd')


def attn_gate_bwd(dg, skip, h, phi, w_theta, b_theta, w_psi, dims, Cs, Ci, dskip, accumulate, dphi, dw_theta, db_theta, dw_psi, db_psi):
    N, D, H, W = dims
    check(lib.vg_attn_gate_bwd(_p(dg), _p(skip), _p(h), _p(phi), _p(w_theta), _p(b_theta), _p(w_psi), N, D, H, W, Cs, Ci,
                               int(skip.dtype == torch.float32), _p(dskip), int(bool(accumulate)), _p(dphi), _p(dw_theta), _p(db_theta),
                               _p(dw_psi), _p(db_psi), stream()), 'vg_attn_gate_bwd')


def tanh_bwd(dy, y, dpre):
    check(lib.vg_tanh_bwd(_p(dy), _p(y), _p(dpre), dy.numel(), stream()), 'vg_tanh_bwd')


def minmax(x, B, S, mm4):
    check(lib.vg_minmax(_p(x), B, S, _p(mm4), stream()), 'vg_minmax')


def minmax_apply(x, mm4, B, S, y):
    check(lib.vg_minmax_apply(_p(x), _p(mm4), B, S, _p(y), stream()), 'vg_minmax_apply')


def minmax_bwd(x, y, gy, mm4, B, S, tmp2, dx):
    check(lib.vg_minmax_bwd(_p(x), _p(y), _p(gy), _p(mm4), B, S, _p(tmp2), _p(dx), stream()), 'vg_minmax_bwd')


def bce(t, p, acc, gscale=0.0, gp=None, accumulate=False):
    check(lib.vg_bce(_p(t), _p(p), t.numel(), _p(acc), gscale, _p(gp), int(accumulate), stream()), 'vg_bce')


def mse(a, b, acc, gscale=0.0, gb=None, accumulate=False):
    check(lib.vg_mse(_p(a), _p(b), a.numel(), _p(acc), gscale, _p(gb), int(accumulate), stream()), 'vg_mse')


def mse_const(x, target, acc, gscale=0.0, gx=None, accumulate=False):
    check(lib.vg_mse_const(_p(x), int(x.dtype == torch.float32), target, x.numel(), _p(acc), gscale, _p(gx),
                           int(accumulate), stream()), 'vg_mse_const')


def lp_loss(a, b, p, acc, gscale=0.0, gb=None, accumulate=False):
    check(lib.vg_lp_loss(_p(a), _p(b), a.numel(), int(p), _p(acc), gscale, _p(gb), int(accumulate), stream()), 'vg_lp_loss')


LOGIT_BCE, LOGIT_FOCAL = 0, 1


def logit_loss(x, target, kind, acc, gscale=0.0, gx=None, accumulate=False):
    check(lib.vg_logit_loss(_p(x), int(x.dtype == torch.float32), target, int(kind), x.numel(), _p(acc), gscale, _p(gx),
                            int(accumulate), stream()), 'vg_logit_loss')


def ssim_fwd(t, p, dims, acc, part):
    B, D, H, W = dims
    check(lib.vg_ssim_fwd(_p(t), _p(p), B, D, H, W, _p(acc), _p(part), stream()), 'vg_ssim_fwd')


def ssim_bwd(t, p, part, dims, gscale, gp, accumulate=False):
    B, D, H, W = dims
    check(lib.vg_ssim_bwd(_p(t), _p(p), _p(part), B, D, H, W, gscale, _p(gp), int(accumulate), stream()), 'vg_ssim_bwd')


def skel_aux_bytes(dims, iters) -> int:
    B, D, H, W = dims
# ... 71 lines not shown
```

Before: 124.7 Mvoxels/s.

## Fuse next block's shortcut norm-backward statistics into producing apply and pointwise kernels

Adds a statistics 'rider' that accumulates the next residual block's shortcut instance-norm backward reductions (sum of grad and sum of grad times normalized x) while the preceding actnorm-apply or 1x1 pointwise dgrad kernel writes that gradient. This removes a separate stats pass that re-reads the full gradient tensor, across encoder blocks, the bridge and the output layer. In exchange the kernels carry extra registers, an extra bf16 input read and shared-memory reductions with atomics, and Python threads a done flag through the block backward.

```diff
diff --git a/include/vangan_hip.h b/include/vangan_hip.h
--- a/include/vangan_hip.h
+++ b/include/vangan_hip.h
@@ -146,6 +146,7 @@
     float* dbeta;
     int32_t* ticket;
     int32_t alias_n0, alias_shift, pgrad_n, pad_;
+    const struct vg_actnorm_bwd_desc_s* out_bstat;
 } vg_actnorm_bwd_desc;
 int vg_actnorm_bwd_stats(const vg_actnorm_bwd_desc* d, vg_stream_t stream);
 int vg_actnorm_bwd_apply(const vg_actnorm_bwd_desc* d, vg_stream_t stream);
diff --git a/van_gan_amd/_lib.py b/van_gan_amd/_lib.py
--- a/van_gan_amd/_lib.py
+++ b/van_gan_amd/_lib.py
@@ -61,7 +61,7 @@
         ('gamma', c_void_p), ('mean', c_void_p), ('rstd', c_void_p), ('red', c_void_p),
         ('dx', c_void_p), ('dx_f32', c_int), ('accumulate', c_int), ('dx_cstride', c_int), ('dx_coff', c_int),
         ('f32', c_int), ('dgamma', c_void_p), ('dbeta', c_void_p), ('ticket', c_void_p),
-        ('alias_n0', c_int), ('alias_shift', c_int), ('pgrad_n', c_int), ('pad_', c_int),
+        ('alias_n0', c_int), ('alias_shift', c_int), ('pgrad_n', c_int), ('pad_', c_int), ('out_bstat', c_void_p),
     ]
 
 
diff --git a/van_gan_amd/csrc/vg_bstat.h b/van_gan_amd/csrc/vg_bstat.h
--- /dev/null
+++ b/van_gan_amd/csrc/vg_bstat.h
@@ -0,0 +1,52 @@
+#pragma once
+#include "vg_common.h"
+
+struct VgBstat {
+    const bf16_t* x;
+    const float* mean; const float* rstd;
+    float* red;
+    int N, C, alias_n0, alias_sh;
+};
+
+static inline bool vg_bstat_ok(const vg_actnorm_bwd_desc* b, const void* out, int N, int D, int H, int W, int C) {
+    if (!b || b->g != out || b->g_padded || !b->norm || b->act != VG_ACT_NONE || b->mult || b->f32 || b->x_f32 || b->x1) return false;
+    if (!b->x || !b->mean || !b->rstd || !b->red) return false;
+    if (b->N != N || b->D != D || b->H != H || b->W != W || b->C != C || (C % 8) || C > 512) return false;
+    if (b->alias_n0 < 0 || (b->alias_n0 > 0 && (b->alias_shift < 1 || b->alias_shift > b->alias_n0 || b->alias_n0 >= N))) return false;
+    return true;
+}
+static inline VgBstat vg_bstat_of(const vg_actnorm_bwd_desc* b) {
+    VgBstat r = {};
+    if (b) { r.x = (const bf16_t*)b->x; r.mean = b->mean; r.rstd = b->rstd; r.red = b->red; r.N = b->N; r.C = b->C;
+             r.alias_n0 = b->alias_n0; r.alias_sh = b->alias_shift; }
+    return r;
+}
+
+#ifdef __HIPCC__
+__device__ __forceinline__ int vg_bstat_nx(const VgBstat& b, int n) { return (b.alias_n0 > 0 && n >= b.alias_n0) ? n - b.alias_sh : n; }
+
+__device__ __forceinline__ void vg_bstat_add8(const float* v, const Raw8<bf16_t>& xr, const float* mu, const float* rs, float* s0, float* s1) {
+    float x[8]; raw_unpack(xr, x);
+#pragma unroll
+    for (int j = 0; j < 8; ++j) {
+        const float dn = bfround(v[j]);
+        s0[j] += dn; s1[j] += dn * ((x[j] - mu[j]) * rs[j]);
+    }
+}
+
+__device__ __forceinline__ void vg_bstat_reduce(const VgBstat& b, int n, int stripe, float* part, const float* s0, const float* s1, bool live,
+                                                int gpc, int vpb) {
+    const int tid = threadIdx.x;
+#pragma unroll
+    for (int j = 0; j < 8; ++j) { part[(2 * j) * 256 + tid] = live ? s0[j] : 0.f; part[(2 * j + 1) * 256 + tid] = live ? s1[j] : 0.f; }
+    __syncthreads();
+    float* dst = b.red + ((size_t)stripe * b.N + n) * b.C * 2;
+    for (int o = tid; o < b.C * 2; o += 256) {
+        const int ch = o >> 1, mom = o & 1, g8 = ch >> 3, j = ch & 7;
+        const float* src = part + (2 * j + mom) * 256 + g8;
+        float a = 0.f;
+        for (int t = 0; t < vpb; ++t) a += src[t * gpc];
+        atomicAdd(&dst[o], a);
+    }
+}
+#endif
diff --git a/van_gan_amd/csrc/vg_common.h b/van_gan_amd/csrc/vg_common.h
--- a/van_gan_amd/csrc/vg_common.h
+++ b/van_gan_amd/csrc/vg_common.h
@@ -142,7 +142,7 @@
     hipError_t e = hipGetLastError();
     return e == hipSuccess ? VG_OK : VG_ELAUNCH;
 }
-int vg_pointwise_conv(const vg_conv_desc* d, hipStream_t s);
+int vg_pointwise_conv(const vg_conv_desc* d, hipStream_t s, bool* did_stats = nullptr);
 int vg_pointwise_wgrad(const vg_conv_desc* d, const void* dy, int dy_f32, int T_total, float* dw, float* db, float* scratch,
                        int64_t scratch_bytes, hipStream_t s);
 int vg_wgrad_dma(const vg_conv_desc* d, const void* dy, int dy_f32, const int32_t* tap_idx_host, int T_total, float* dw, float* db,
diff --git a/van_gan_amd/csrc/vg_conv.hip b/van_gan_amd/csrc/vg_conv.hip
--- a/van_gan_amd/csrc/vg_conv.hip
+++ b/van_gan_amd/csrc/vg_conv.hip
@@ -910,7 +910,7 @@
 static int conv3d_impl(const vg_conv_desc* d, vg_stream_t stream, bool& did_stats) {
     if (d && d->wlayout) return vg_conv_dma(d, (hipStream_t)stream, &did_stats);
     if (d && d->out && d->wpacked && d->src0 && !d->res_c1) {
-        const int prc = vg_pointwise_conv(d, (hipStream_t)stream);
+        const int prc = vg_pointwise_conv(d, (hipStream_t)stream, &did_stats);
         if (prc <= 0) return prc;
     }
     GatherIn g; ConvOut k; ConvCls q; int BN, MSUB, lds;
diff --git a/van_gan_amd/csrc/vg_elem.hip b/van_gan_amd/csrc/vg_elem.hip
--- a/van_gan_amd/csrc/vg_elem.hip
+++ b/van_gan_amd/csrc/vg_elem.hip
@@ -1,4 +1,5 @@
 #include "vg_common.h"
+#include "vg_bstat.h"
 #include <stdlib.h>
 
 __global__ void in_finalize_kernel(const float* sums0, int c0, float cnt0, const float* sums1, int c1, float cnt1,
@@ -52,6 +53,7 @@
     void* dx; int dx_f32, accumulate, dx_cstride, dx_coff;
     int gpc, vpb;
     int alias_n0, alias_sh, pgrad_n;
+    VgBstat ob;
 };
 __device__ __forceinline__ int anb_nx(const ANB& p, int n) { return (p.alias_n0 > 0 && n >= p.alias_n0) ? n - p.alias_sh : n; }
 
@@ -81,8 +83,9 @@
 template <typename T> __device__ __forceinline__ void rawv_unpack(const RawV<T, 8>& o, float* v) { raw_unpack(o.r, v); }
 template <typename T> __device__ __forceinline__ void rawv_unpack(const RawV<T, 1>& o, float* v) { v[0] = o.r; }
 
-template <typename T, int VEC, int UB, typename F>
-__device__ __forceinline__ void anb_walk_from(const ANB& p, int n, int c, int v, const int stride, const ChanK<VEC>& ck, F&& consume) {
+template <typename T, int VEC, int UB, bool EX = false, typename F>
+__device__ __forceinline__ void anb_walk_from(const ANB& p, int n, int c, int v, const int stride, const ChanK<VEC>& ck, F&& consume,
+                                              const bf16_t* ex = nullptr) {
     const int S = p.D * p.H * p.W;
     if (v >= S) return;
     int w = v % p.W, t0 = v / p.W; int h = t0 % p.H, d = t0 / p.H;
@@ -101,6 +104,7 @@
     const void* x1p = (const char*)p.x + (size_t)nx * S * (p.x_f32 ? 4 : 2);
     for (; v < S; v += UB * stride) {
         RawV<T, VEC> gr[UB], xr[UB];
+        Raw8<bf16_t> er[EX ? UB : 1];
         float x1v[UB];
         int vv[UB], dd[UB], hh[UB], ww[UB];
 #pragma unroll
@@ -112,6 +116,7 @@
             const int dc = ok ? d : dd[0], hc = ok ? h : hh[0], wc = ok ? w : ww[0];
             const size_t gi = p.g_padded ? ((size_t)((dc + 1) * PH + hc + 1) * PW + wc + 1) * p.C : (size_t)vc * p.C;
             rawv_load(gr[k], gp + gi);
+            if constexpr (EX) { if (ex) raw_load(er[k], ex + (size_t)vc * p.C); }
             if (need_x) {
                 if (VEC == 8) {
                     const size_t xi = cat0 ? ((size_t)((dc >> xs) * Hs + (hc >> xs)) * Ws + (wc >> xs)) * cx : (size_t)vc * cx;
@@ -186,14 +191,14 @@
                 } else xh[j] = 0.f;
                 dn[j] = gv;
             }
-            consume(vv[k], dn, xh);
+            consume(vv[k], dn, xh, er[EX ? k : 0]);
         }
     }
 }
 
 template <typename T, int VEC, int UB, typename F>
 __device__ __forceinline__ void anb_walk(const ANB& p, int n, int c, int vl, const ChanK<VEC>& ck, F&& consume) {
-    anb_walk_from<T, VEC, UB>(p, n, c, (int)(blockIdx.x * p.vpb + vl), (int)(gridDim.x * p.vpb), ck, consume);
+    anb_walk_from<T, VEC, UB, false>(p, n, c, (int)(blockIdx.x * p.vpb + vl), (int)(gridDim.x * p.vpb), ck, consume);
 }
 
 template <typename T, int VEC>
@@ -210,7 +215,7 @@
     if (tid < nthr) {
         ChanK<VEC> ck;
         load_chank<VEC>(p, n, cg * VEC, ck);
-        anb_walk<T, VEC, 4>(p, n, cg * VEC, vl, ck, [&](int, const float* dn, const float* xh) {
+        anb_walk<T, VEC, 4>(p, n, cg * VEC, vl, ck, [&](int, const float* dn, const float* xh, const Raw8<bf16_t>&) {
 #pragma unroll
             for (int j = 0; j < VEC; ++j) { s0[j] += dn[j]; s1[j] += dn[j] * xh[j]; }
         });
@@ -232,15 +237,28 @@
     for (int i = tid; i < p.C * 2; i += 256) atomicAdd(&dst[i], red[i]);
 }
 
-template <typename T, int VEC>
-__device__ __forceinline__ void actnorm_apply_body(const ANB& p, const int bx, const int gx) {
+template <typename T, int VEC, bool RIDER>
+__device__ __forceinline__ void actnorm_apply_body(const ANB& p, const int bx, const int gx, float* part) {
     const int n = blockIdx.y;
     const int tid = threadIdx.x;
     const int nthr = p.gpc * p.vpb;
-    if (tid >= nthr) return;
+    const bool live = tid < nthr;
+    if (!RIDER && !live) return;
     const int cg = tid % p.gpc, vl = tid / p.gpc;
     const int S = p.D * p.H * p.W;
     const int c = cg * VEC;
+    float b0[RIDER ? 8 : 1], b1[RIDER ? 8 : 1], bmu[RIDER ? 8 : 1], brs[RIDER ? 8 : 1];
+    const bf16_t* ex = nullptr;
+    if constexpr (RIDER) {
+#pragma unroll
+        for (int j = 0; j < 8; ++j) { b0[j] = 0.f; b1[j] = 0.f; bmu[j] = 0.f; brs[j] = 0.f; }
+        if (p.ob.red && live) {
+            const int nx = vg_bstat_nx(p.ob, n);
+            ldvec(p.ob.mean + nx * p.C + c, bmu, 8); ldvec(p.ob.rstd + nx * p.C + c, brs, 8);
+            ex = p.ob.x + (size_t)nx * S * p.C + c;
+        }
+    }
+    if (live) {
     float k0[VEC], k1[VEC], k2[VEC];
 #pragma unroll
     for (int j = 0; j < VEC; ++j) { k0[j] = 1.f; k1[j] = 0.f; k2[j] = 0.f; }
@@ -269,7 +287,7 @@
     }
     ChanK<VEC> ck;
     load_chank<VEC>(p, n, c, ck);
-    anb_walk_from<T, VEC, 4>(p, n, c, bx * p.vpb + vl, gx * p.vpb, ck, [&](int v, const float* dn, const float* xh) {
+    anb_walk_from<T, VEC, 4, RIDER>(p, n, c, bx * p.vpb + vl, gx * p.vpb, ck, [&](int v, const float* dn, const float* xh, const Raw8<bf16_t>& er) {
         float o[VEC];
 #pragma unroll
         for (int j = 0; j < VEC; ++j) o[j] = k0[j] * dn[j] - k1[j] - k2[j] * xh[j];
@@ -286,18 +304,34 @@
                 for (int j = 0; j < 8; ++j) o[j] += old[j];
             }
             store8<bf16_t>(q, o);
+            if constexpr (RIDER) { if (ex) vg_bstat_add8(o, er, bmu, brs, b0, b1); }
         } else {
             bf16_t* q = (bf16_t*)p.dx + oidx;
             q[0] = f2bf(p.accumulate ? bf2f(q[0]) + o[0] : o[0]);
         }
-    });
-}
-template <typename T, int VEC>
-__global__ __launch_bounds__(256) void actnorm_apply_kernel(const ANB p) { actnorm_apply_body<T, VEC>(p, (int)blockIdx.x, (int)gridDim.x); }
-template <typename T, int VEC>
+    }, ex);
+    }
+    if constexpr (RIDER) {
+        if (p.ob.red) vg_bstat_reduce(p.ob, n, bx & (VG_STRIPES - 1), part, b0, b1, live, p.gpc, p.vpb);
+    }
+}
+template <typename T, int VEC, bool RIDER = false>
+__global__ __launch_bounds__(256) void actnorm_apply_kernel(const ANB p) {
+    if constexpr (RIDER) {
+        __shared__ float part[16 * 256];
+        actnorm_apply_body<T, VEC, true>(p, (int)blockIdx.x, (int)gridDim.x, part);
+    } else actnorm_apply_body<T, VEC, false>(p, (int)blockIdx.x, (int)gridDim.x, nullptr);
+}
+template <typename T, int VEC, bool RIDER = false>
 __global__ __launch_bounds__(256) void actnorm_apply2_kernel(const ANB p1, const ANB p2, const int g1) {
-    if ((int)blockIdx.x < g1) actnorm_apply_body<T, VEC>(p1, (int)blockIdx.x, g1);
-    else actnorm_apply_body<T, VEC>(p2, (int)blockIdx.x - g1, (int)gridDim.x - g1);
+    if constexpr (RIDER) {
+        __shared__ float part[16 * 256];
+        if ((int)blockIdx.x < g1) actnorm_apply_body<T, VEC, true>(p1, (int)blockIdx.x, g1, part);
+        else actnorm_apply_body<T, VEC, true>(p2, (int)blockIdx.x - g1, (int)gridDim.x - g1, part);
+    } else {
+        if ((int)blockIdx.x < g1) actnorm_apply_body<T, VEC, false>(p1, (int)blockIdx.x, g1, nullptr);
+        else actnorm_apply_body<T, VEC, false>(p2, (int)blockIdx.x - g1, (int)gridDim.x - g1, nullptr);
+    }
 }
 
 static int fill_anb(const vg_actnorm_bwd_desc* d, ANB& p, bool apply) {
@@ -318,6 +352,7 @@
     p.dx = d->dx; p.dx_f32 = (d->dx_f32 || d->f32) ? 1 : 0; p.accumulate = d->accumulate;
     p.dx_cstride = d->dx_cstride > 0 ? d->dx_cstride : d->C; p.dx_coff = d->dx_coff;
     p.alias_n0 = d->alias_n0; p.alias_sh = d->alias_shift; p.pgrad_n = d->pgrad_n;
+    p.ob = VgBstat{};
     if (d->alias_n0 < 0 || (d->alias_n0 > 0 && (d->alias_shift < 1 || d->alias_shift > d->alias_n0 || d->alias_n0 >= d->N)) || d->pgrad_n < 0) return VG_EINVAL;
     p.gpc = d->C == 1 ? 1 : d->C / 8;
     if (p.gpc > 256 || d->C > 512) return VG_EINVAL;
@@ -349,10 +384,25 @@
     }
     return vg_check_launch();
 }
+static int anb_rider(const vg_actnorm_bwd_desc* d, ANB& p) {
+    const vg_actnorm_bwd_desc* ob = d->out_bstat;
+    if (!ob) return 0;
+    if (ob->g != d->dx) return VG_EINVAL;
+    if (d->f32 || p.dx_f32 || p.C == 1 || p.dx_cstride != p.C || p.dx_coff != 0 || !vg_bstat_ok(ob, d->dx, d->N, d->D, d->H, d->W, d->C)) return 0;
+    p.ob = vg_bstat_of(ob);
+    return 1;
+}
 extern "C" int vg_actnorm_bwd_apply(const vg_actnorm_bwd_desc* d, vg_stream_t stream) {
     vg_begin();
     ANB p; int rc = fill_anb(d, p, true);
     if (rc != VG_OK) return rc;
+    const int ride = anb_rider(d, p);
+    if (ride < 0) return ride;
+    if (ride) {
+        hipLaunchKernelGGL((actnorm_apply_kernel<bf16_t, 8, true>), anb_grid(p), dim3(256), 0, (hipStream_t)stream, p);
+        return vg_check_launch();
+    }
+    const int done = d->out_bstat ? 2 : VG_OK;
     if (d->f32) {
         if (p.C == 1) hipLaunchKernelGGL((actnorm_apply_kernel<float, 1>), anb_grid(p), dim3(256), 0, (hipStream_t)stream, p);
         else hipLaunchKernelGGL((actnorm_apply_kernel<float, 8>), anb_grid(p), dim3(256), 0, (hipStream_t)stream, p);
@@ -360,7 +410,8 @@
         if (p.C == 1) hipLaunchKernelGGL((actnorm_apply_kernel<bf16_t, 1>), anb_grid(p), dim3(256), 0, (hipStream_t)stream, p);
         else hipLaunchKernelGGL((actnorm_apply_kernel<bf16_t, 8>), anb_grid(p), dim3(256), 0, (hipStream_t)stream, p);
     }
-    return vg_check_launch();
+    rc = vg_check_launch();
+    return rc == VG_OK ? done : rc;
 }
 
 extern "C" int vg_actnorm_bwd_apply2(const vg_actnorm_bwd_desc* d1, const vg_actnorm_bwd_desc* d2, vg_stream_t stream) {
@@ -370,10 +421,25 @@
     rc = fill_anb(d2, p2, true); if (rc != VG_OK) return rc;
     if (!vg_tune("ANB_APPLY2", 1) || d1->N != d2->N || (d1->f32 != 0) != (d2->f32 != 0) || d1->C == 1 || d2->C == 1) {
         rc = vg_actnorm_bwd_apply(d1, stream);
-        return rc != VG_OK ? rc : vg_actnorm_bwd_apply(d2, stream);
+        if (rc < 0) return rc;
+        const int rc2 = vg_actnorm_bwd_apply(d2, stream);
+        return rc2 < 0 ? rc2 : (rc | rc2);
     }
     const dim3 g1 = anb_grid(p1), g2 = anb_grid(p2);
     const dim3 grid(g1.x + g2.x, g1.y);
+    if (d1->out_bstat || d2->out_bstat) {
+        const int r1 = anb_rider(d1, p1), r2 = anb_rider(d2, p2);
+        if (r1 < 0 || r2 < 0) return VG_EINVAL;
+        if ((d1->out_bstat && !r1) || (d2->out_bstat && !r2)) { p1.ob = VgBstat{}; p2.ob = VgBstat{}; }
+        else {
+            hipLaunchKernelGGL((actnorm_apply2_kernel<bf16_t, 8, true>), grid, dim3(256), 0, (hipStream_t)stream, p1, p2, (int)g1.x);
+            return vg_check_launch();
+        }
+        if (d1->f32) hipLaunchKernelGGL((actnorm_apply2_kernel<float, 8>), grid, dim3(256), 0, (hipStream_t)stream, p1, p2, (int)g1.x);
+        else hipLaunchKernelGGL((actnorm_apply2_kernel<bf16_t, 8>), grid, dim3(256), 0, (hipStream_t)stream, p1, p2, (int)g1.x);
+        rc = vg_check_launch();
+        return rc == VG_OK ? 2 : rc;
+    }
     if (d1->f32) hipLaunchKernelGGL((actnorm_apply2_kernel<float, 8>), grid, dim3(256), 0, (hipStream_t)stream, p1, p2, (int)g1.x);
     else hipLaunchKernelGGL((actnorm_apply2_kernel<bf16_t, 8>), grid, dim3(256), 0, (hipStream_t)stream, p1, p2, (int)g1.x);
     return vg_check_launch();
diff --git a/van_gan_amd/csrc/vg_pointwise.hip b/van_gan_amd/csrc/vg_pointwise.hip
--- a/van_gan_amd/csrc/vg_pointwise.hip
+++ b/van_gan_amd/csrc/vg_pointwise.hip
@@ -1,5 +1,6 @@
 #include "vg_common.h"
 #include "vg_c1k3.h"
+#include "vg_bstat.h"
 #include <stdlib.h>
 
 namespace {
@@ -15,6 +16,7 @@
     float* dw; float* db;
     int N, C; int64_t S;
     VgFin fin;
+    VgBstat bs;
 };
 
 __device__ __forceinline__ float pw_slope(int act) { return act == VG_ACT_RELU ? 0.f : (act == VG_ACT_LRELU ? VG_LRELU : 1.f); }
@@ -79,8 +81,9 @@
     }
 }
 
-template <typename T>
+template <typename T, bool BS = false>
 __global__ __launch_bounds__(256) void pw_1toc_kernel(const PW p) {
+    static_assert(!BS || sizeof(T) == 2, "the statistics rider reads and writes the 16-bit storage type");
     __shared__ float part[16 * 256];
     const int n = blockIdx.y, tid = threadIdx.x;
     const int gpc = p.C >> 3, vpb = 256 / gpc;
@@ -97,14 +100,26 @@
     const int64_t xoff = (int64_t)n * p.S;
     T* ob = (T*)p.out + (size_t)n * p.S * p.C + cg * 8;
     const int64_t stride = (int64_t)gridDim.x * vpb;
+    float b0[8], b1[8], bmu[8], brs[8];
+    const bf16_t* bx = nullptr;
+    if constexpr (BS) {
+        const int nx = vg_bstat_nx(p.bs, n);
+#pragma unroll
+        for (int j = 0; j < 8; ++j) {
+            b0[j] = 0.f; b1[j] = 0.f;
+            bmu[j] = live ? p.bs.mean[nx * p.C + cg * 8 + j] : 0.f; brs[j] = live ? p.bs.rstd[nx * p.C + cg * 8 + j] : 0.f;
+        }
+        bx = p.bs.x + (size_t)nx * p.S * p.C + cg * 8;
+    }
     if (live)
     for (int64_t v = (int64_t)blockIdx.x * vpb + vl; v < p.S; v += 4 * stride) {
-        float xs[4]; Raw8<T> old[4];
+        float xs[4]; Raw8<T> old[4]; Raw8<bf16_t> bxr[BS ? 4 : 1];
 #pragma unroll
         for (int k = 0; k < 4; ++k) {
             const int64_t vv = v + k * stride < p.S ? v + k * stride : v;
             xs[k] = ld_single(p.x, p.x_f32, xoff + vv);
             if (p.accumulate) raw_load(old[k], ob + vv * p.C);
+            if constexpr (BS) raw_load(bxr[k], bx + vv * p.C);
         }
 #pragma unroll
         for (int k = 0; k < 4; ++k) {
@@ -122,7 +137,12 @@
             store8<T>(ob + (v + k * stride) * p.C, o);
 #pragma unroll
             for (int j = 0; j < 8; ++j) { const float r = rnd<T>(o[j]); s1[j] += r; s2[j] += r * r; }
-        }
+            if constexpr (BS) vg_bstat_add8(o, bxr[k], bmu, brs, b0, b1);
+        }
+    }
+    if constexpr (BS) {
+        vg_bstat_reduce(p.bs, n, blockIdx.x & (VG_STRIPES - 1), part, b0, b1, live, gpc, vpb);
+        if (p.sums) __syncthreads();
     }
     if (!p.sums) return;
 #pragma unroll
@@ -1005,7 +1025,7 @@
     return pw_gemm_split(d, b, dlow, dskip, c_low, accumulate, (hipStream_t)stream);
 }
 
-int vg_pointwise_conv(const vg_conv_desc* d, hipStream_t s) {
+int vg_pointwise_conv(const vg_conv_desc* d, hipStream_t s, bool* did_stats) {
     if (pw_enabled() && !d->res && !d->tanh_out && !d->accumulate && d->ostr == 1 && !d->ooff_d && !d->ooff_h && !d->ooff_w
         && d->BD == d->OD && d->BH == d->OH && d->BW == d->OW && !(d->out_f32 && !d->f32)) {
         { const int mrc = c1m_fwd(d, s); if (mrc <= 0) return mrc; }
@@ -1062,7 +1082,14 @@
         const dim3 grid(pw_blocks((p.S + 3) / 4 * (256 / vpb), d->N), d->N);
         if (vg_dry("pw_1toc<%s>", d->f32 ? "f32" : "bf16")) return VG_OK;
         p.fin = vg_fin_of(d);
-        if (d->f32) hipLaunchKernelGGL((pw_1toc_kernel<float>), grid, dim3(256), 0, s, p);
+        const bool ride = did_stats && !d->f32 && !d->out_f32 && !d->accumulate
+                          && vg_bstat_ok(d->bstat, d->out, d->N, d->D, d->H, d->W, d->Cout);
+        if (ride) {
+            p.bs = vg_bstat_of(d->bstat);
+            hipLaunchKernelGGL((pw_1toc_kernel<bf16_t, true>), grid, dim3(256), 0, s, p);
+            *did_stats = true;
+        }
+        else if (d->f32) hipLaunchKernelGGL((pw_1toc_kernel<float>), grid, dim3(256), 0, s, p);
         else hipLaunchKernelGGL((pw_1toc_kernel<bf16_t>), grid, dim3(256), 0, s, p);
         if (p.sums && p.fin.ticket) vg_fin_done = true;
         return vg_check_launch();
diff --git a/van_gan_amd/nets.py b/van_gan_amd/nets.py
--- a/van_gan_amd/nets.py
+++ b/van_gan_amd/nets.py
@@ -459,20 +459,36 @@
     def _norm_bwd(self, ar, g, g_padded, src: Src, st, norm: Norm, dx, act, dx_cstride=0, accumulate=True):
         ops.actnorm_run(self._norm_desc(ar, g, g_padded, src, st, norm, dx, act, dx_cstride, accumulate))
 
-    def _dgrad_norm_bwd(self, ar, lay, dy, N, dp, src: Src, st, norm: Norm, dx, act, accumulate):
+    def _dgrad_norm_bwd(self, ar, lay, dy, N, dp, src: Src, st, norm: Norm, dx, act, accumulate, out_bstat=None) -> bool:
         dsc = self._norm_desc(ar, dp, True, src, st, norm, dx, act, accumulate=accumulate)
-        ops.actnorm_run(dsc, stats_done=lay.dgrad(dy, N, dp, accumulate=False, bstat=dsc))
-
-    def _block_bwd(self, ar: Arena, name: str, c: dict, N: int, inline: bool = False):
+        if out_bstat is not None:
+            ops.actnorm_set_out_bstat(dsc, out_bstat)
+        return ops.actnorm_run(dsc, stats_done=lay.dgrad(dy, N, dp, accumulate=False, bstat=dsc))
+
+    def _short_desc(self, ar: Arena, name: str, c: dict, N: int):
+        sc = c['sc']
+        ssc = Src(sc.data, (N,) + sc.dims, sc.C)
+        c['dsc1'] = self._norm_desc(ar, c['out'].grad, False, ssc, c['ns'], self.Nn[name + '.short'], None, ACT_NONE, accumulate=False)
+        c['dsc1_done'] = False
+        return c['dsc1']
+
+    def _rider_ok(self) -> bool:
+        return ops.SHORTCUT_BSTAT and ops.DRY is None and self.dtype != torch.float32 and not self.attention_gate
+
+    def _block_bwd(self, ar: Arena, name: str, c: dict, N: int, inline: bool = False, nxt: Optional[dict] = None, nxt_name: str = ''):
         L, Nn = self.L, self.Nn
         out, r, sc = c['out'], c['r'], c['sc']
         d_out = out.grad
         cb1, cb2, short = L[name + '.cb1'], L[name + '.cb2'], L[name + '.short']
+        ndsc = self._short_desc(ar, nxt_name, nxt, N) if (nxt is not None and self._rider_ok()) else None
         mk = ar.mark()
         d_sc = ar.alloc(sc.data.shape, self.dtype)
-        ssc = Src(sc.data, (N,) + sc.dims, sc.C)
-        dsc1 = self._norm_desc(ar, d_out, False, ssc, c['ns'], Nn[name + '.short'], d_sc, ACT_NONE, accumulate=False)
-        ops.actnorm_stats(dsc1)
+        dsc1 = c.get('dsc1')
+        if dsc1 is None:
+            dsc1 = self._short_desc(ar, name, c, N)
+        ops.actnorm_set_dx(dsc1, d_sc)
+        if not c['dsc1_done']:
+            ops.actnorm_stats(dsc1)
         cb2.wgrad(c['s2'], d_out, inline)
         dp = ar.alloc((N,) + cb2.buf_dims + (r.C,), self.dtype)
         d_r = ar.alloc(r.data.shape, self.dtype)
@@ -488,8 +504,13 @@
         if len(inp) == 1:
             gin = inp[0].alloc_grad(ar) if inp[0].grad is None else inp[0].grad
             assert inp[0].grad_init, 'encoder input gradient must have had its first (overwriting) writer: the decoder skip path'
-            self._dgrad_norm_bwd(ar, cb1, d_r, N, dp1, s1, c['n1'], Nn[name + '.cb1'], gin, ACT_RELU, accumulate=True)
-            short.dgrad(d_sc, N, gin, accumulate=True)
+            if ndsc is None:
+                self._dgrad_norm_bwd(ar, cb1, d_r, N, dp1, s1, c['n1'], Nn[name + '.cb1'], gin, ACT_RELU, accumulate=True)
+                short.dgrad(d_sc, N, gin, accumulate=True)
+            else:
+                short.dgrad(d_sc, N, gin, accumulate=True)
+                nxt['dsc1_done'] = self._dgrad_norm_bwd(ar, cb1, d_r, N, dp1, s1, c['n1'], Nn[name + '.cb1'], gin, ACT_RELU, accumulate=True,
+                                                        out_bstat=ndsc)
         else:
             low, skip = inp
             dsc = self._norm_desc(ar, dp1, True, s1, c['n1'], Nn[name + '.cb1'], None, ACT_RELU, accumulate=False)
@@ -517,6 +538,9 @@
         for a in acts:
             a.grad = None
             a.alloc_grad(ar)
+        for k in ['enc%d' % e for e in range(1, 5)] + ['dec%d' % d for d in range(4)]:
+            ctx[k].pop('dsc1', None)
+            ctx[k]['dsc1_done'] = False
         dpre = ar.alloc(gy.shape, torch.float32)
         if isinstance(ctx['y'], list):
             nb = N // len(ctx['y'])
@@ -526,12 +550,18 @@
             ops.tanh_bwd(gy, ctx['y'], dpre)
         h = ctx['out']['inp']
         L['out'].wgrad(ctx['out']['so'], dpre)
-        L['out'].dgrad(dpre, N, h.grad, accumulate=not h.first_write())
+        first = h.first_write()
+        c0 = ctx['dec0']
+        if first and self._rider_ok():
+            c0['dsc1_done'] = L['out'].dgrad(dpre, N, h.grad, accumulate=False, bstat=self._short_desc(ar, 'dec0', c0, N))
+        else:
+            L['out'].dgrad(dpre, N, h.grad, accumulate=not first)
         for d in (0, 1, 2, 3):
             self._block_bwd(ar, 'dec%d' % d, ctx['dec%d' % d], N)
             if self.attention_gate:
                 self._gate_bwd(ar, d, ctx['dec%d' % d], N)
         b = ctx['bridge']
+        pre4 = self._short_desc(ar, 'enc4', ctx['enc4'], N) if self._rider_ok() else None
         mk = ar.mark()
         cb2, cb1 = L['bridge.cb2'], L['bridge.cb1']
         cb2.wgrad(b['sb2'], b['b2'].grad)
@@ -540,10 +570,13 @@
         self._dgrad_norm_bwd(ar, cb2, b['b2'].grad, N, dp, b['sb2'], b['nb2'], Nn['bridge.cb2'], d_b1, ACT_RELU, accumulate=False)
         cb1.wgrad(b['sb1'], d_b1)
         dp = ar.alloc((N,) + cb1.buf_dims + (b['inp'].C,), self.dtype)
-        self._dgrad_norm_bwd(ar, cb1, d_b1, N, dp, b['sb1'], b['nb1'], Nn['bridge.cb1'], b['inp'].grad, ACT_RELU, accumulate=not b['inp'].first_write())
+        c4 = ctx['enc4']
+        c4['dsc1_done'] = self._dgrad_norm_bwd(ar, cb1, d_b1, N, dp, b['sb1'], b['nb1'], Nn['bridge.cb1'], b['inp'].grad, ACT_RELU,
+                                               accumulate=not b['inp'].first_write(), out_bstat=pre4)
         ar.release(mk, defer=True)
         for e in (4, 3, 2, 1):
-            self._block_bwd(ar, 'enc%d' % e, ctx['enc%d' % e], N, inline=e <= inline_from)
+            self._block_bwd(ar, 'enc%d' % e, ctx['enc%d' % e], N, inline=e <= inline_from,
+                            nxt=ctx['enc%d' % (e - 1)] if e > 1 else None, nxt_name='enc%d' % (e - 1))
             if e == 4 and on_suffix_done is not None:
                 on_suffix_done()
         inl = inline_from >= 0
diff --git a/van_gan_amd/ops.py b/van_gan_amd/ops.py
--- a/van_gan_amd/ops.py
+++ b/van_gan_amd/ops.py
@@ -292,6 +292,7 @@
 FUSE_CONCAT = os.environ.get('VG_FUSE_CONCAT', '1') != '0'
 BSTAT = os.environ.get('VG_BSTAT', '1') != '0'
 BSTAT_DMA = os.environ.get('VG_BSTAT_DMA', '0') != '0'
+SHORTCUT_BSTAT = os.environ.get('VG_SHORTCUT_BSTAT', '1') != '0'
 SIDE: Optional[bool] = None
 _SIDE_OF = {}
 
@@ -884,7 +885,9 @@
         use_bs = bstat is not None and BSTAT and not accumulate and not self.f32 and out.dtype in (torch.bfloat16, torch.float16) and bstat.norm \
             and ((len(self.d_classes) == 1 and self.stride == 1 and self.k == 3 and self.pad == 'reflect'
                   and self.d_classes[0]['ck'] == 16 and self.cin % 16 == 0 and self.cout % 16 == 0 and not bstat.mult)
-                 or (bool(self.d_bn) and BSTAT_DMA))
+                 or (bool(self.d_bn) and BSTAT_DMA)
+                 or (SHORTCUT_BSTAT and DRY is None and self.k == 1 and self.cout == 1 and self.stride == 1 and self.cin % 8 == 0
+                     and not self.d_fused and len(self.d_classes) == 1 and not bstat.g_padded and bstat.act == ACT_NONE and not bstat.mult))
         if DRY is not None:
             DRY.tag = ('dgrad', self.name)
             DRY.recipe = dict(kind='dgrad', layer=self.ctor, N=N, accumulate=bool(accumulate), dy_f32=dy.dtype == torch.float32,
@@ -1206,15 +1209,24 @@
     d._keep = d._keep + (dx,)
 
 
-def actnorm_run(d: ActNormBwdDesc, stats_done: bool = False):
+def actnorm_set_out_bstat(d: ActNormBwdDesc, ob: Optional[ActNormBwdDesc]):
+    d.out_bstat = None if ob is None else C.addressof(ob)
+    d._keep = d._keep + (ob,)
+    if REC is not None and ob is not None:
+        REC.keep.append(ob)
+
+
+def actnorm_run(d: ActNormBwdDesc, stats_done: bool = False) -> bool:
     if stats_done:
-        check(lib.vg_actnorm_bwd_apply(C.byref(d), stream()), 'vg_actnorm_bwd_apply')
+        rc = check(lib.vg_actnorm_bwd_apply(C.byref(d), stream()), 'vg_actnorm_bwd_apply')
     else:
-        check(lib.vg_actnorm_bwd(C.byref(d), stream()), 'vg_actnorm_bwd')
-
-
-def actnorm_apply2(d1: ActNormBwdDesc, d2: ActNormBwdDesc):
-    check(lib.vg_actnorm_bwd_apply2(C.byref(d1), C.byref(d2), stream()), 'vg_actnorm_bwd_apply2')
+        rc = check(lib.vg_actnorm_bwd(C.byref(d), stream()), 'vg_actnorm_bwd')
+    return bool(d.out_bstat) and rc == 0
+
+
+def actnorm_apply2(d1: ActNormBwdDesc, d2: ActNormBwdDesc) -> bool:
+    rc = check(lib.vg_actnorm_bwd_apply2(C.byref(d1), C.byref(d2), stream()), 'vg_actnorm_bwd_apply2')
+    return bool(d1.out_bstat or d2.out_bstat) and rc == 0
 
 
 def actnorm_bwd(g, g_padded, x, dims, C_, dx, **kw):
```

Measured after the change: 125.2 Mvoxels/s, median of 6. No clear change (+0.3%).
